# IrisRainbowNeko/HCP-Diffusion

Hardware: NVIDIA H100
Metric: LoRA-train images/sec SD1.5 512px (higher is better)
Workload: dtype bf16

## Files before the change

hcp_diffusion_b200/csrc/attention.cu:

```cuda
#include <stdlib.h>
#include "common.cuh"
#include "host_util.h"
#include "../../include/hcp_b200.h"

namespace hcp {

constexpr int kAttnThreads = 288;
constexpr int kAttnBwdThreads = 256;
constexpr int BOX_BYTES = 128 * 128;
constexpr float kLog2e = 1.4426950408889634f;
constexpr float kLn2 = 0.6931471805599453f;

__device__ __forceinline__ uint32_t kmajor_off(int ks, int box_bytes) { return (uint32_t)((ks >> 2) * (box_bytes >> 4) + (ks & 3) * 2); }
__device__ __forceinline__ float quad_max(float v) {
    v = fmaxf(v, __shfl_xor_sync(0xffffffffu, v, 1));
    return fmaxf(v, __shfl_xor_sync(0xffffffffu, v, 2));
}
__device__ __forceinline__ float quad_sum(float v) {
    v += __shfl_xor_sync(0xffffffffu, v, 1);
    return v + __shfl_xor_sync(0xffffffffu, v, 2);
}

struct alignas(64) AttnFwdParams {
    CUtensorMap tmQ, tmK, tmV;
    int B, H, Lq, Lkv, d;
    int nks;
    float scale_log2;
    const float* kv_bias;
    __nv_bfloat16* O;
    int64_t ldo;
    float* lse;
};

template <int NB, int KVT>
struct AttnFwdCfg {
    static constexpr int Q_BYTES = NB * BOX_BYTES;
    static constexpr int KV_BOX = KVT * 128;
    static constexpr int KV_BYTES = NB * KV_BOX;
    static constexpr int STAGES = 2;
    static constexpr int SMEM_BYTES = Q_BYTES + 2 * STAGES * KV_BYTES + 256 + 1024;
};

template <int NB, int KVT, bool kCausal>
__global__ void __launch_bounds__(kAttnThreads, 1) attn_fwd_kernel(const __grid_constant__ AttnFwdParams p) {
    using Cfg = AttnFwdCfg<NB, KVT>;
    constexpr int STAGES = Cfg::STAGES;
    constexpr int DN = 64 * NB;
    extern __shared__ uint8_t smem_raw[];
    uint8_t* smem = reinterpret_cast<uint8_t*>((reinterpret_cast<uintptr_t>(smem_raw) + 1023) & ~uintptr_t(1023));
    uint8_t* sQ = smem;
    uint8_t* sK = sQ + Cfg::Q_BYTES;
    uint8_t* sV = sK + STAGES * Cfg::KV_BYTES;
    uint64_t* bars = reinterpret_cast<uint64_t*>(sV + STAGES * Cfg::KV_BYTES);
    uint64_t* q_full = bars;
    uint64_t* kv_full = bars + 1;
    uint64_t* kv_empty = bars + 1 + STAGES;

    const int warp = warp_id_uniform(), lane = threadIdx.x & 31;
    const int qt = blockIdx.x, h = blockIdx.y, b = blockIdx.z;
    const int nkv = kCausal ? min((p.Lkv + KVT - 1) / KVT, (qt * 128 + 128 + KVT - 1) / KVT) : (p.Lkv + KVT - 1) / KVT;

    if (threadIdx.x == 0) {
        mbar_init(q_full, 1);
        for (int s = 0; s < STAGES; ++s) { mbar_init(&kv_full[s], 1); mbar_init(&kv_empty[s], 256); }
        fence_mbar_init();
    }
    __syncthreads();
    pdl_trigger();
    pdl_wait();

    if (warp == 8) {
        if (elect_one()) {
            mbar_arrive_expect_tx(q_full, Cfg::Q_BYTES);
            for (int bx = 0; bx < NB; ++bx) tma_load_4d(sQ + bx * BOX_BYTES, &p.tmQ, q_full, bx * 64, h, qt * 128, b);
            for (int j = 0; j < nkv; ++j) {
                const int st = j % STAGES;
                mbar_wait(&kv_empty[st], ((j / STAGES) & 1) ^ 1);
                mbar_arrive_expect_tx(&kv_full[st], 2 * Cfg::KV_BYTES);
                for (int bx = 0; bx < NB; ++bx) {
                    tma_load_4d(sK + st * Cfg::KV_BYTES + bx * Cfg::KV_BOX, &p.tmK, &kv_full[st], bx * 64, h, j * KVT, b);
                    tma_load_4d(sV + st * Cfg::KV_BYTES + bx * Cfg::KV_BOX, &p.tmV, &kv_full[st], bx * 64, h, j * KVT, b);
                }
            }
        }
        return;
    }

    const int wg = warp >> 2;
    const int g = lane >> 2, cq = 2 * (lane & 3);
    const int row0 = wg * 64 + (warp & 3) * 16 + g;
    const float* bias = p.kv_bias ? p.kv_bias + (int64_t)b * p.Lkv : nullptr;
    const float sl2 = p.scale_log2;
    float m[2] = {-INFINITY, -INFINITY}, l[2] = {0.f, 0.f};
    float o[DN / 2];
#pragma unroll
    for (int i = 0; i < DN / 2; ++i) o[i] = 0.f;
    const uint64_t qdesc = make_smem_desc(smem_u32(sQ) + wg * 64 * 128, 16, 1024);
    mbar_wait(q_full, 0);
    for (int j = 0; j < nkv; ++j) {
        const int st = j % STAGES;
        const int kv0 = j * KVT;
        const int ncols = min(KVT, p.Lkv - kv0);
        mbar_wait(&kv_full[st], (j / STAGES) & 1);
        float s[KVT / 2];
        const uint64_t kdesc = make_smem_desc(smem_u32(sK + st * Cfg::KV_BYTES), 16, 1024);
        wgmma_fence();
        wgmma_ss<KVT, 0, 0>(s, qdesc, kdesc, 0u);
        for (int ks = 1; ks < p.nks; ++ks)
            wgmma_ss<KVT, 0, 0>(s, desc_adv(qdesc, kmajor_off(ks, BOX_BYTES)), desc_adv(kdesc, kmajor_off(ks, Cfg::KV_BOX)), 1u);
        wgmma_commit();
        wgmma_wait<0>();
        wgmma_fence_acc(s);
        float mx[2] = {-INFINITY, -INFINITY};
        const bool diag = kCausal && kv0 + KVT > qt * 128;
#pragma unroll
        for (int c8 = 0; c8 < KVT / 8; ++c8) {
#pragma unroll
            for (int e = 0; e < 2; ++e) {
                const int col = c8 * 8 + cq + e;
                const float bv = (bias && col < ncols) ? bias[kv0 + col] * kLog2e : 0.f;
#pragma unroll
                for (int hh = 0; hh < 2; ++hh) {
                    float v = s[4 * c8 + 2 * hh + e] * sl2 + bv;
                    v = (col < ncols) ? v : -INFINITY;
                    if (diag && kv0 + col > qt * 128 + row0 + 8 * hh) v = -INFINITY;
                    s[4 * c8 + 2 * hh + e] = v;
                    mx[hh] = fmaxf(mx[hh], v);
                }
            }
        }
        float mu[2];
#pragma unroll
        for (int hh = 0; hh < 2; ++hh) {
            const float m_new = fmaxf(m[hh], quad_max(mx[hh]));
            mu[hh] = (m_new == -INFINITY) ? 0.f : m_new;
            const float alpha = fast_exp2(m[hh] - mu[hh]);
            l[hh] *= alpha;
#pragma unroll
            for (int c8 = 0; c8 < DN / 8; ++c8) { o[4 * c8 + 2 * hh] *= alpha; o[4 * c8 + 2 * hh + 1] *= alpha; }
            m[hh] = m_new;
        }
        uint32_t pa[KVT / 16][4];
#pragma unroll
        for (int kk = 0; kk < KVT / 16; ++kk) {
#pragma unroll
            for (int r = 0; r < 4; ++r) {
                const int hh = r & 1;
                const int i = 8 * kk + 4 * (r >> 1) + 2 * hh;
                const uint32_t u = pack_bf16x2(fast_exp2(s[i] - mu[hh]), fast_exp2(s[i + 1] - mu[hh]));
                const float2 f = unpack_bf16x2(u);
                l[hh] += f.x + f.y;
                pa[kk][r] = u;
            }
        }
        const uint64_t vdesc = make_smem_desc(smem_u32(sV + st * Cfg::KV_BYTES), Cfg::KV_BOX, 1024);
        wgmma_fence();
#pragma unroll
        for (int kk = 0; kk < KVT / 16; ++kk) wgmma_rs<DN, 1>(o, pa[kk], desc_adv(vdesc, kk * 128), 1u);
        wgmma_commit();
        wgmma_wait<0>();
        wgmma_fence_acc(o);
        mbar_arrive(&kv_empty[st]);
    }
#pragma unroll
    for (int hh = 0; hh < 2; ++hh) {
        const float lt = quad_sum(l[hh]);
        const int qrow = qt * 128 + row0 + 8 * hh;
        if (qrow >= p.Lq) continue;
        const float inv = 1.f / lt;
        __nv_bfloat16* orow = p.O + ((int64_t)b * p.Lq + qrow) * p.ldo + (int64_t)h * p.d;
#pragma unroll
        for (int c8 = 0; c8 < DN / 8; ++c8) {
            const int col = c8 * 8 + cq;
            if (col < p.d) *reinterpret_cast<uint32_t*>(orow + col) = pack_bf16x2(o[4 * c8 + 2 * hh] * inv, o[4 * c8 + 2 * hh + 1] * inv);
        }
        if (cq == 0 && p.lse) p.lse[((int64_t)b * p.H + h) * p.Lq + qrow] = ((m[hh] == -INFINITY ? 0.f : m[hh]) + log2f(lt)) * kLn2;
    }
}

struct alignas(64) AttnBwdParams {
    CUtensorMap tmQ, tmK, tmV, tmdO;
    int B, H, Lq, Lkv, d;
    int nks;
    int col0;
    float scale, scale_log2;
    const float* kv_bias;
    const float* stats;
    float* dq_acc;
    int dq_ld;
    int qsplit;
    float* dkv_acc;
    __nv_bfloat16 *dK, *dV;
    int64_t lddk, lddv;
};

template <int NB>
struct AttnBwdCfg {
    static constexpr int KV_BYTES = NB * BOX_BYTES;
    static constexpr int QBOX = 64 * 128;
    static constexpr int Q_BYTES = NB * QBOX;
    static constexpr int STAGES = 2;
    static constexpr int DS_BYTES = 64 * 128;
    static constexpr int STAT_BYTES = 2 * 64 * 4;
    static constexpr int SMEM_BYTES = 2 * KV_BYTES + 2 * STAGES * Q_BYTES + 2 * DS_BYTES + STAGES * STAT_BYTES + 256 + 1024;
};

template <int NB, bool kCausal>
__global__ void __launch_bounds__(kAttnBwdThreads, 1) attn_bwd_kernel(const __grid_constant__ AttnBwdParams p) {
    using Cfg = AttnBwdCfg<NB>;
    constexpr int STAGES = Cfg::STAGES;
    extern __shared__ uint8_t smem_raw[];
    uint8_t* smem = reinterpret_cast<uint8_t*>((reinterpret_cast<uintptr_t>(smem_raw) + 1023) & ~uintptr_t(1023));
    uint8_t* sK = smem;
    uint8_t* sV = sK + Cfg::KV_BYTES;
    uint8_t* sQ = sV + Cfg::KV_BYTES;
    uint8_t* sdO = sQ + STAGES * Cfg::Q_BYTES;
    uint8_t* sDS = sdO + STAGES * Cfg::Q_BYTES;
    uint8_t* sStat = sDS + 2 * Cfg::DS_BYTES;
    uint64_t* bars = reinterpret_cast<uint64_t*>(sStat + STAGES * Cfg::STAT_BYTES);
    uint64_t* kv_full = bars;
    uint64_t* q_full = bars + 1;

    const int warp = warp_id_uniform(), lane = threadIdx.x & 31;
    const int kt = blockIdx.x / p.qsplit, qs = blockIdx.x % p.qsplit;
    const int h = blockIdx.y, b = blockIdx.z;
    const int nq = (p.Lq + 63) / 64;
    const int per = 2 * (((nq + 1) / 2 + p.qsplit - 1) / p.qsplit);
    const int i0 = kCausal ? max(qs * per, 2 * kt) : qs * per, i1 = min(nq, qs * per + per);
    if (kCausal && i0 >= i1) return;
    const int64_t bh = (int64_t)b * p.H + h;

    if (threadIdx.x == 0) {
        mbar_init(kv_full, 1);
        for (int s = 0; s < STAGES; ++s) mbar_init(&q_full[s], 1);
        fence_mbar_init();
    }
    __syncthreads();
    pdl_trigger();
    pdl_wait();

    auto load_q = [&](int i) {
        const int st = (i - i0) % STAGES;
        mbar_arrive_expect_tx(&q_full[st], 2 * Cfg::Q_BYTES + Cfg::STAT_BYTES);
        for (int bx = 0; bx < NB; ++bx) {
            tma_load_4d(sQ + st * Cfg::Q_BYTES + bx * Cfg::QBOX, &p.tmQ, &q_full[st], bx * 64, h, i * 64, b);
            tma_load_4d(sdO + st * Cfg::Q_BYTES + bx * Cfg::QBOX, &p.tmdO, &q_full[st], bx * 64, h, i * 64, b);
        }
        bulk_load(sStat + st * Cfg::STAT_BYTES, p.stats + (bh * nq + i) * 128, Cfg::STAT_BYTES, &q_full[st]);
    };
    if (threadIdx.x == 0) {
        mbar_arrive_expect_tx(kv_full, 2 * Cfg::KV_BYTES);
        for (int bx = 0; bx < NB; ++bx) {
            tma_load_4d(sK + bx * BOX_BYTES, &p.tmK, kv_full, bx * 64, h, kt * 128, b);
            tma_load_4d(sV + bx * BOX_BYTES, &p.tmV, kv_full, bx * 64, h, kt * 128, b);
        }
        for (int i = i0; i < min(i1, i0 + STAGES); ++i) load_q(i);
    }

    const int wg = warp >> 2;
    const int g = lane >> 2, cq = 2 * (lane & 3);
    const int r0 = (warp & 3) * 16 + g;
    const int kvw = kt * 128 + wg * 64;
    const float sl2 = p.scale_log2, scale = p.scale;
    const int cbox = p.col0 / 64;
    float kvb[2];
    bool kv_ok[2];
#pragma unroll
    for (int hh = 0; hh < 2; ++hh) {
        const int kv = kvw + r0 + 8 * hh;
        kv_ok[hh] = kv < p.Lkv;
        kvb[hh] = (p.kv_bias && kv_ok[hh]) ? p.kv_bias[(int64_t)b * p.Lkv + kv] * kLog2e : 0.f;
    }
    float dv[32], dk[32];
#pragma unroll
    for (int i = 0; i < 32; ++i) { dv[i] = 0.f; dk[i] = 0.f; }
    const uint64_t kdesc = make_smem_desc(smem_u32(sK) + wg * 64 * 128, 16, 1024);
    const uint64_t vdesc = make_smem_desc(smem_u32(sV) + wg * 64 * 128, 16, 1024);
    const int dq_col = p.col0 + 32 * wg;
    const bool dq_cols = dq_col < p.d;
    const uint64_t kdesc_mn = make_smem_desc(smem_u32(sK) + cbox * BOX_BYTES + wg * 64, BOX_BYTES, 1024);
    const uint32_t ds_base = smem_u32(sDS) + wg * Cfg::DS_BYTES;
    const uint64_t dsdesc = make_smem_desc(smem_u32(sDS), 2 * Cfg::DS_BYTES, 1024);
    mbar_wait(kv_full, 0);
    for (int i = i0; i < i1; ++i) {
        const int st = (i - i0) % STAGES;
        mbar_wait(&q_full[st], ((i - i0) / STAGES) & 1);
        const uint32_t qb = smem_u32(sQ + st * Cfg::Q_BYTES), dob = smem_u32(sdO + st * Cfg::Q_BYTES);
        const uint32_t statb = smem_u32(sStat + st * Cfg::STAT_BYTES);
        const uint64_t qdesc = make_smem_desc(qb, 16, 1024), dodesc = make_smem_desc(dob, 16, 1024);
        float s[32], dp[32];
        wgmma_fence();
        wgmma_ss<64, 0, 0>(s, kdesc, qdesc, 0u);
        for (int ks = 1; ks < p.nks; ++ks)
            wgmma_ss<64, 0, 0>(s, desc_adv(kdesc, kmajor_off(ks, BOX_BYTES)), desc_adv(qdesc, kmajor_off(ks, Cfg::QBOX)), 1u);
        wgmma_ss<64, 0, 0>(dp, vdesc, dodesc, 0u);
        for (int ks = 1; ks < p.nks; ++ks)
            wgmma_ss<64, 0, 0>(dp, desc_adv(vdesc, kmajor_off(ks, BOX_BYTES)), desc_adv(dodesc, kmajor_off(ks, Cfg::QBOX)), 1u);
        wgmma_commit();
        wgmma_wait<0>();
        wgmma_fence_acc(s);
        wgmma_fence_acc(dp);
        uint32_t pa[4][4], da[4][4];
        const bool diag = kCausal && i < 2 * kt + 2;
#pragma unroll
        for (int kk = 0; kk < 4; ++kk) {
            float lq[4], dq_[4];
#pragma unroll
            for (int c2 = 0; c2 < 2; ++c2) {
                const uint32_t a = statb + (16 * kk + 8 * c2 + cq) * 4;
                const float2 l2 = lds_f32x2(a), d2 = lds_f32x2(a + 64 * 4);
                lq[2 * c2] = l2.x; lq[2 * c2 + 1] = l2.y;
                dq_[2 * c2] = d2.x; dq_[2 * c2 + 1] = d2.y;
            }
#pragma unroll
            for (int r = 0; r < 4; ++r) {
                const int hh = r & 1;
                const int c = 2 * (r >> 1);
                const int idx = 8 * kk + 4 * (r >> 1) + 2 * hh;
                float pv[2], dsv[2];
#pragma unroll
                for (int e = 0; e < 2; ++e) {
                    float pe = kv_ok[hh] ? fast_exp2(s[idx + e] * sl2 + kvb[hh] - lq[c + e]) : 0.f;
                    if (diag && kvw + r0 + 8 * hh > i * 64 + 16 * kk + 8 * (r >> 1) + cq + e) pe = 0.f;
                    pv[e] = pe;
                    dsv[e] = scale * pe * (dp[idx + e] - dq_[c + e]);
                }
                pa[kk][r] = pack_bf16x2(pv[0], pv[1]);
                da[kk][r] = pack_bf16x2(dsv[0], dsv[1]);
                const int row = r0 + 8 * hh, col = 16 * kk + 8 * (r >> 1) + cq;
                asm volatile("st.shared.b32 [%0], %1;" ::"r"(ds_base + sw128_offset(row, col >> 3) + (col & 7) * 2), "r"(da[kk][r]) : "memory");
            }
        }
        fence_proxy_async_smem();
        asm volatile("bar.sync 1, 256;" ::: "memory");
        const uint64_t dodesc_mn = make_smem_desc(dob + cbox * Cfg::QBOX, Cfg::QBOX, 1024);
        const uint64_t qdesc_mn = make_smem_desc(qb + cbox * Cfg::QBOX, Cfg::QBOX, 1024);
        float dqa[16];
        wgmma_fence();
#pragma unroll
        for (int kk = 0; kk < 4; ++kk) wgmma_rs<64, 1>(dv, pa[kk], desc_adv(dodesc_mn, kk * 128), 1u);
#pragma unroll
        for (int kk = 0; kk < 4; ++kk) wgmma_rs<64, 1>(dk, da[kk], desc_adv(qdesc_mn, kk * 128), 1u);
        if (dq_cols) {
            wgmma_ss<32, 1, 1>(dqa, dsdesc, kdesc_mn, 0u);
#pragma unroll
            for (int kk = 1; kk < 8; ++kk) wgmma_ss<32, 1, 1>(dqa, desc_adv(dsdesc, kk * 128), desc_adv(kdesc_mn, kk * 128), 1u);
        }
        wgmma_commit();
        wgmma_wait<0>();
        wgmma_fence_acc(dv);
        wgmma_fence_acc(dk);
        wgmma_fence_acc(dqa);
        asm volatile("bar.sync 1, 256;" ::: "memory");
        if (threadIdx.x == 0 && i + STAGES < i1) load_q(i + STAGES);
        if (!dq_cols) continue;
#pragma unroll
        for (int hh = 0; hh < 2; ++hh) {
            const int q = i * 64 + r0 + 8 * hh;
            if (q >= p.Lq) continue;
#pragma unroll
            for (int c8 = 0; c8 < 4; ++c8) {
                const int col = dq_col + 8 * c8 + cq;
                if (col < p.d) red_add_v2(p.dq_acc + ((bh * (p.dq_ld / 4) + col / 4) * p.Lq + q) * 4 + (col & 3), dqa[4 * c8 + 2 * hh], dqa[4 * c8 + 2 * hh + 1]);
            }
        }
    }
#pragma unroll
    for (int hh = 0; hh < 2; ++hh) {
        if (!kv_ok[hh]) continue;
        const int kv = kvw + r0 + 8 * hh;
#pragma unroll
        for (int c8 = 0; c8 < 8; ++c8) {
            const int col = p.col0 + 8 * c8 + cq;
            if (col >= p.d) continue;
            const float v0 = dv[4 * c8 + 2 * hh], v1 = dv[4 * c8 + 2 * hh + 1];
            const float k0 = dk[4 * c8 + 2 * hh], k1 = dk[4 * c8 + 2 * hh + 1];
            if (p.dkv_acc) {
                float* base = p.dkv_acc + ((bh * p.Lkv + kv) * 2) * p.dq_ld + col;
                red_add_v2(base, v0, v1);
                red_add_v2(base + p.dq_ld, k0, k1);
            } else {
                *reinterpret_cast<uint32_t*>(p.dV + ((int64_t)b * p.Lkv + kv) * p.lddv + (int64_t)h * p.d + col) = pack_bf16x2(v0, v1);
                *reinterpret_cast<uint32_t*>(p.dK + ((int64_t)b * p.Lkv + kv) * p.lddk + (int64_t)h * p.d + col) = pack_bf16x2(k0, k1);
            }
        }
    }
}

__global__ void __launch_bounds__(256) attn_bwd_prep_kernel(const __nv_bfloat16* __restrict__ O, int64_t ldo,
                                                            const __nv_bfloat16* __restrict__ dO, int64_t lddo,
                                                            const float* __restrict__ lse, int B, int H, int Lq, int d,
                                                            float* __restrict__ stats, float* __restrict__ dq_acc,
                                                            int64_t dq_n, float* __restrict__ dkv_acc, int64_t dkv_n) {
    pdl_trigger();
    pdl_wait();
    const int64_t gtid = blockIdx.x * (int64_t)blockDim.x + threadIdx.x;
    const int64_t nthreads = (int64_t)gridDim.x * blockDim.x;
    if (dq_acc) {
        float4* z = reinterpret_cast<float4*>(dq_acc);
        for (int64_t i = gtid; i < dq_n / 4; i += nthreads) z[i] = make_float4(0.f, 0.f, 0.f, 0.f);
    }
    if (dkv_acc) {
        float4* z = reinterpret_cast<float4*>(dkv_acc);
        for (int64_t i = gtid; i < dkv_n / 4; i += nthreads) z[i] = make_float4(0.f, 0.f, 0.f, 0.f);
    }
    const int nq = (Lq + 63) / 64;
    const int64_t total = (int64_t)B * nq * 64 * H;
    if (gtid >= total) return;
    const int h = (int)(gtid % H);
    const int64_t bq = gtid / H;
    const int q = (int)(bq % (nq * 64));
    const int b = (int)(bq / (nq * 64));
    float* st = stats + (((int64_t)b * H + h) * nq + q / 64) * 128 + (q & 63);
    if (q >= Lq) {
        st[0] = INFINITY;
        st[64] = 0.f;
        return;
    }
    const int64_t row = (int64_t)b * Lq + q;
    const uint4* o = reinterpret_cast<const uint4*>(O + row * ldo + (int64_t)h * d);
    const uint4* g = reinterpret_cast<const uint4*>(dO + row * lddo + (int64_t)h * d);
    float acc = 0.f;
    for (int e = 0; e < d / 8; ++e) {
        const uint4 a = o[e], c = g[e];
        float2 x, y;
        x = unpack_bf16x2(a.x); y = unpack_bf16x2(c.x); acc += x.x * y.x + x.y * y.y;
        x = unpack_bf16x2(a.y); y = unpack_bf16x2(c.y); acc += x.x * y.x + x.y * y.y;
        x = unpack_bf16x2(a.z); y = unpack_bf16x2(c.z); acc += x.x * y.x + x.y * y.y;
        x = unpack_bf16x2(a.w); y = unpack_bf16x2(c.w); acc += x.x * y.x + x.y * y.y;
    }
    st[0] = lse[((int64_t)b * H + h) * Lq + q] * kLog2e;
    st[64] = acc;
}

__global__ void attn_bwd_post_kernel(const float* __restrict__ dq_acc, int dq_ld, int B, int H, int Lq, int d,
                                     __nv_bfloat16* __restrict__ dQ, int64_t lddq) {
    pdl_trigger();
    pdl_wait();
    const int64_t i = blockIdx.x * (int64_t)blockDim.x + threadIdx.x;
    const int d4 = d / 4;
    const int64_t total = (int64_t)B * Lq * H * d4;
    if (i >= total) return;
    const int e = (int)(i % d4) * 4;
    const int64_t r = i / d4;
    const int h = (int)(r % H);
    const int64_t bq = r / H;
    const int q = (int)(bq % Lq);
    const int b = (int)(bq / Lq);
    const float4 v = *reinterpret_cast<const float4*>(dq_acc + ((((int64_t)b * H + h) * (dq_ld / 4) + e / 4) * Lq + q) * 4);
    uint2 o;
    o.x = pack_bf16x2(v.x, v.y);
    o.y = pack_bf16x2(v.z, v.w);
    *reinterpret_cast<uint2*>(dQ + bq * lddq + (int64_t)h * d + e) = o;
}

__global__ void attn_bwd_post_kv_kernel(const float* __restrict__ acc, int dq_ld, int B, int H, int Lkv, int d,
                                        __nv_bfloat16* __restrict__ dK, int64_t lddk, __nv_bfloat16* __restrict__ dV, int64_t lddv) {
    pdl_trigger();
    pdl_wait();
    const int64_t i = blockIdx.x * (int64_t)blockDim.x + threadIdx.x;
    const int d4 = d / 4;
    const int64_t total = (int64_t)B * Lkv * H * 2 * d4;
    if (i >= total) return;
    const int e = (int)(i % d4) * 4;
    int64_t r = i / d4;
    const int which = (int)(r % 2); r /= 2;
    const int h = (int)(r % H);
    const int64_t bk = r / H;
    const int kv = (int)(bk % Lkv);
    const int b = (int)(bk / Lkv);
    const float4 v = *reinterpret_cast<const float4*>(acc + ((((int64_t)b * H + h) * Lkv + kv) * 2 + which) * dq_ld + e);
    uint2 o;
    o.x = pack_bf16x2(v.x, v.y);
    o.y = pack_bf16x2(v.z, v.w);
    __nv_bfloat16* dst = which ? dK : dV;
    const int64_t ld = which ? lddk : lddv;
    *reinterpret_cast<uint2*>(dst + bk * ld + (int64_t)h * d + e) = o;
}

static int make_head_map(CUtensorMap* m, const void* base, int64_t ld, int64_t B, int64_t H, int64_t L, int64_t d, uint32_t rows) {
    uint64_t dims[4] = {(uint64_t)d, (uint64_t)H, (uint64_t)L, (uint64_t)B};
    uint64_t strides[3] = {(uint64_t)d * 2, (uint64_t)ld * 2, (uint64_t)L * ld * 2};
    uint32_t box[4] = {64, 1, rows, 1};
    return make_tmap_nd(m, base, 4, dims, strides, box);
}

static int check_common(int64_t B, int64_t H, int64_t Lq, int64_t Lkv, int64_t d) {
    if (B <= 0 || H <= 0 || Lq <= 0 || Lkv <= 0) return set_error(HCP_ERR_INVALID, "attention: empty problem");
    if (d % 8 != 0 || d < 8 || d > 192) return set_error(HCP_ERR_INVALID, "attention: head dim must be a multiple of 8 in [8,192]");
    return HCP_OK;
}

template <int NB, int KVT, bool kCausal>
static int launch_attn_fwd(const AttnFwdParams& p, dim3 grid, cudaStream_t stream) {
    using Cfg = AttnFwdCfg<NB, KVT>;
    static bool configured = false;
    if (!configured) {
        cudaError_t e = cudaFuncSetAttribute(attn_fwd_kernel<NB, KVT, kCausal>, cudaFuncAttributeMaxDynamicSharedMemorySize, Cfg::SMEM_BYTES);
        if (e != cudaSuccess) return set_cuda_error(e, "cudaFuncSetAttribute(attn_fwd)");
        configured = true;
    }
    launch_k(attn_fwd_kernel<NB, KVT, kCausal>, grid, dim3(kAttnThreads), Cfg::SMEM_BYTES, stream, p);
    cudaError_t e = cudaGetLastError();
    if (e != cudaSuccess) return set_cuda_error(e, "attn_fwd launch");
    return HCP_OK;
}

template <int NB, bool kCausal>
static int launch_attn_bwd(const AttnBwdParams& p, dim3 grid, cudaStream_t stream) {
    using Cfg = AttnBwdCfg<NB>;
    static bool configured = false;
    if (!configured) {
        cudaError_t e = cudaFuncSetAttribute(attn_bwd_kernel<NB, kCausal>, cudaFuncAttributeMaxDynamicSharedMemorySize, Cfg::SMEM_BYTES);
        if (e != cudaSuccess) return set_cuda_error(e, "cudaFuncSetAttribute(attn_bwd)");
        configured = true;
    }
    launch_k(attn_bwd_kernel<NB, kCausal>, grid, dim3(kAttnBwdThreads), Cfg::SMEM_BYTES, stream, p);
    cudaError_t e = cudaGetLastError();
    if (e != cudaSuccess) return set_cuda_error(e, "attn_bwd launch");
    return HCP_OK;
}

}

using namespace hcp;

template <bool kCausal>
static int attn_fwd(const hcp_attn_args* a, hcp_stream_t stream_) {
    if (!a || !a->q || !a->k || !a->v || !a->o) return set_error(HCP_ERR_INVALID, "attn_fwd: null pointer");
    int rc = check_common(a->B, a->H, a->Lq, a->Lkv, a->d);
    if (rc) return rc;
    if (kCausal && a->Lq != a->Lkv) return set_error(HCP_ERR_INVALID, "attn_fwd_causal: Lq must equal Lkv");
    const int nb = (int)((a->d + 63) / 64);
    const uint32_t kvt = nb == 3 ? 64 : 128;
    AttnFwdParams p;
    memset(&p, 0, sizeof(p));
    if ((rc = make_head_map(&p.tmQ, a->q, a->ldq, a->B, a->H, a->Lq, a->d, 128))) return rc;
    if ((rc = make_head_map(&p.tmK, a->k, a->ldk, a->B, a->H, a->Lkv, a->d, kvt))) return rc;
    if ((rc = make_head_map(&p.tmV, a->v, a->ldv, a->B, a->H, a->Lkv, a->d, kvt))) return rc;
    p.B = (int)a->B; p.H = (int)a->H; p.Lq = (int)a->Lq; p.Lkv = (int)a->Lkv; p.d = (int)a->d;
    p.nks = (int)((a->d + 15) / 16);
    p.scale_log2 = a->scale * kLog2e;
    p.kv_bias = a->kv_bias;
    p.O = (__nv_bfloat16*)a->o; p.ldo = a->ldo;
    p.lse = a->lse;
    const dim3 grid((unsigned)((a->Lq + 127) / 128), (unsigned)a->H, (unsigned)a->B);
    cudaStream_t stream = (cudaStream_t)stream_;
    if (nb == 1) return launch_attn_fwd<1, 128, kCausal>(p, grid, stream);
    if (nb == 2) return launch_attn_fwd<2, 128, kCausal>(p, grid, stream);
    return launch_attn_fwd<3, 64, kCausal>(p, grid, stream);
}

extern "C" int hcp_attn_fwd_bf16(const hcp_attn_args* a, hcp_stream_t stream) { return attn_fwd<false>(a, stream); }
extern "C" int hcp_attn_fwd_causal_bf16(const hcp_attn_args* a, hcp_stream_t stream) { return attn_fwd<true>(a, stream); }

static int plan_qsplit(int64_t B, int64_t H, int64_t Lq, int64_t Lkv) {
    const int64_t base = ((Lkv + 127) / 128) * H * B;
    const int64_t nq = (Lq + 127) / 128;
    const int64_t sms = num_sms();
    if (base >= sms * 4 / 5 || nq < 2) return 1;
    int64_t qs = (2 * sms + base - 1) / base;
    if (qs > nq) qs = nq;
    const int64_t per = (nq + qs - 1) / qs;
    return (int)((nq + per - 1) / per);
}

extern "C" size_t hcp_attn_bwd_workspace_bytes(int64_t B, int64_t H, int64_t Lq, int64_t Lkv, int64_t d) {
    const int64_t dq_ld = (d + 3) / 4 * 4;
    size_t n = (size_t)(B * H * ((Lq + 63) / 64) * 128) + (size_t)(B * H * Lq * dq_ld);
    if (plan_qsplit(B, H, Lq, Lkv) > 1) n += (size_t)(B * H * Lkv * 2 * dq_ld);
    return n * sizeof(float);
}

template <bool kCausal>
static int attn_bwd(const hcp_attn_bwd_args* a, hcp_stream_t stream_) {
    if (!a || !a->q || !a->k || !a->v || !a->o || !a->dout || !a->lse || !a->dq || !a->dk || !a->dv || !a->workspace)
        return set_error(HCP_ERR_INVALID, "attn_bwd: null pointer");
    int rc = check_common(a->B, a->H, a->Lq, a->Lkv, a->d);
    if (rc) return rc;
    if (kCausal && a->Lq != a->Lkv) return set_error(HCP_ERR_INVALID, "attn_bwd_causal: Lq must equal Lkv");
    if (a->workspace_bytes < hcp_attn_bwd_workspace_bytes(a->B, a->H, a->Lq, a->Lkv, a->d))
        return set_error(HCP_ERR_INVALID, "attn_bwd: workspace too small");
    if ((a->ldo % 8) != 0 || (a->lddo % 8) != 0 || (a->lddq % 8) != 0) return set_error(HCP_ERR_INVALID, "attn_bwd: leading dimensions must be multiples of 8");
    cudaStream_t stream = (cudaStream_t)stream_;
    const int dq_ld = (int)((a->d + 3) / 4 * 4);
    float* stats = a->workspace;
    float* dq_acc = a->workspace + a->B * a->H * ((a->Lq + 63) / 64) * 128;
    const int qsplit = plan_qsplit(a->B, a->H, a->Lq, a->Lkv);
    const int64_t dkv_n = qsplit > 1 ? a->B * a->H * a->Lkv * 2 * dq_ld : 0;
    float* dkv_acc = qsplit > 1 ? dq_acc + a->B * a->H * a->Lq * dq_ld : nullptr;
    {
        const int64_t total = a->B * ((a->Lq + 63) / 64 * 64) * a->H;
        const int threads = 256;
        const int64_t blocks = (total + threads - 1) / threads;
        launch_k(attn_bwd_prep_kernel, dim3((unsigned)blocks), dim3(threads), 0, stream, (const __nv_bfloat16*)a->o, a->ldo,
                 (const __nv_bfloat16*)a->dout, a->lddo, (const float*)a->lse, (int)a->B, (int)a->H, (int)a->Lq, (int)a->d, stats,
                 dq_acc, (int64_t)(a->B * a->H * a->Lq * dq_ld), dkv_acc, dkv_n);
    }
    AttnBwdParams p;
    memset(&p, 0, sizeof(p));
    if ((rc = make_head_map(&p.tmQ, a->q, a->ldq, a->B, a->H, a->Lq, a->d, 64))) return rc;
    if ((rc = make_head_map(&p.tmK, a->k, a->ldk, a->B, a->H, a->Lkv, a->d, 128))) return rc;
    if ((rc = make_head_map(&p.tmV, a->v, a->ldv, a->B, a->H, a->Lkv, a->d, 128))) return rc;
    if ((rc = make_head_map(&p.tmdO, a->dout, a->lddo, a->B, a->H, a->Lq, a->d, 64))) return rc;
    p.B = (int)a->B; p.H = (int)a->H; p.Lq = (int)a->Lq; p.Lkv = (int)a->Lkv; p.d = (int)a->d;
    p.nks = (int)((a->d + 15) / 16);
    p.scale = a->scale;
    p.scale_log2 = a->scale * kLog2e;
    p.kv_bias = a->kv_bias;
    p.stats = stats;
    p.dq_acc = dq_acc;
    p.dq_ld = dq_ld;
    p.qsplit = qsplit;
    p.dkv_acc = dkv_acc;
    p.dK = (__nv_bfloat16*)a->dk; p.lddk = a->lddk;
    p.dV = (__nv_bfloat16*)a->dv; p.lddv = a->lddv;
    const int nb = (int)((a->d + 63) / 64);
    const dim3 grid((unsigned)(((a->Lkv + 127) / 128) * qsplit), (unsigned)a->H, (unsigned)a->B);
    for (int col0 = 0; col0 < a->d; col0 += 64) {
        p.col0 = col0;
        rc = nb == 1 ? launch_attn_bwd<1, kCausal>(p, grid, stream) : nb == 2 ? launch_attn_bwd<2, kCausal>(p, grid, stream)
                     : launch_attn_bwd<3, kCausal>(p, grid, stream);
        if (rc) return rc;
    }
    {
        const int64_t n = a->B * a->Lq * a->H * (a->d / 4);
        launch_k(attn_bwd_post_kernel, dim3((unsigned)((n + 255) / 256)), dim3(256), 0, stream, dq_acc, dq_ld, (int)a->B, (int)a->H, (int)a->Lq,
                 (int)a->d, (__nv_bfloat16*)a->dq, a->lddq);
    }
    if (qsplit > 1) {
        const int64_t n = a->B * a->Lkv * a->H * 2 * (a->d / 4);
        launch_k(attn_bwd_post_kv_kernel, dim3((unsigned)((n + 255) / 256)), dim3(256), 0, stream, dkv_acc, dq_ld, (int)a->B, (int)a->H, (int)a->Lkv, (int)a->d,
                                                                                (__nv_bfloat16*)a->dk, a->lddk, (__nv_bfloat16*)a->dv, a->lddv);
    }
    cudaError_t e = cudaGetLastError();
    if (e != cudaSuccess) return set_cuda_error(e, "attn_bwd post launch");
    return HCP_OK;
}

extern "C" int hcp_attn_bwd_bf16(const hcp_attn_bwd_args* a, hcp_stream_t stream) { return attn_bwd<false>(a, stream); }
extern "C" int hcp_attn_bwd_causal_bf16(const hcp_attn_bwd_args* a, hcp_stream_t stream) { return attn_bwd<true>(a, stream); }
```

hcp_diffusion_b200/csrc/wgmma.cuh:

```cuda
#pragma once
#include <stdint.h>

namespace hcp {
template <int TA, int TB>
__device__ __forceinline__ void wgmma_ss_n32(float (&d)[16], uint64_t a, uint64_t b, uint32_t accumulate) {
    asm volatile(
        "{\n\t.reg .pred p;\n\t"
        "setp.ne.b32 p, %18, 0;\n\t"
        "wgmma.mma_async.sync.aligned.m64n32k16.f32.bf16.bf16 "
        "{%0, %1, %2, %3, %4, %5, %6, %7, %8, %9, %10, %11, %12, %13, %14, %15}, "
        "%16, %17, p, 1, 1, %19, %20;\n\t}"
        : "+f"(d[0]), "+f"(d[1]), "+f"(d[2]), "+f"(d[3]), "+f"(d[4]), "+f"(d[5]), "+f"(d[6]), "+f"(d[7]), "+f"(d[8]), "+f"(d[9]), "+f"(d[10]), "+f"(d[11]), "+f"(d[12]), "+f"(d[13]), "+f"(d[14]), "+f"(d[15])
        : "l"(a), "l"(b), "r"(accumulate), "n"(TA), "n"(TB));
}
template <int TA, int TB>
__device__ __forceinline__ void wgmma_ss_n64(float (&d)[32], uint64_t a, uint64_t b, uint32_t accumulate) {
    asm volatile(
        "{\n\t.reg .pred p;\n\t"
        "setp.ne.b32 p, %34, 0;\n\t"
        "wgmma.mma_async.sync.aligned.m64n64k16.f32.bf16.bf16 "
        "{%0, %1, %2, %3, %4, %5, %6, %7, %8, %9, %10, %11, %12, %13, %14, %15, %16, %17, %18, %19, %20, %21, %22, %23, %24, %25, %26, %27, %28, %29, %30, %31}, "
        "%32, %33, p, 1, 1, %35, %36;\n\t}"
        : "+f"(d[0]), "+f"(d[1]), "+f"(d[2]), "+f"(d[3]), "+f"(d[4]), "+f"(d[5]), "+f"(d[6]), "+f"(d[7]), "+f"(d[8]), "+f"(d[9]), "+f"(d[10]), "+f"(d[11]), "+f"(d[12]), "+f"(d[13]), "+f"(d[14]), "+f"(d[15]), "+f"(d[16]), "+f"(d[17]), "+f"(d[18]), "+f"(d[19]), "+f"(d[20]), "+f"(d[21]), "+f"(d[22]), "+f"(d[23]), "+f"(d[24]), "+f"(d[25]), "+f"(d[26]), "+f"(d[27]), "+f"(d[28]), "+f"(d[29]), "+f"(d[30]), "+f"(d[31])
        : "l"(a), "l"(b), "r"(accumulate), "n"(TA), "n"(TB));
}
template <int TA, int TB>
__device__ __forceinline__ void wgmma_ss_n128(float (&d)[64], uint64_t a, uint64_t b, uint32_t accumulate) {
    asm volatile(
        "{\n\t.reg .pred p;\n\t"
        "setp.ne.b32 p, %66, 0;\n\t"
        "wgmma.mma_async.sync.aligned.m64n128k16.f32.bf16.bf16 "
        "{%0, %1, %2, %3, %4, %5, %6, %7, %8, %9, %10, %11, %12, %13, %14, %15, %16, %17, %18, %19, %20, %21, %22, %23, %24, %25, %26, %27, %28, %29, %30, %31, %32, %33, %34, %35, %36, %37, %38, %39, %40, %41, %42, %43, %44, %45, %46, %47, %48, %49, %50, %51, %52, %53, %54, %55, %56, %57, %58, %59, %60, %61, %62, %63}, "
        "%64, %65, p, 1, 1, %67, %68;\n\t}"
        : "+f"(d[0]), "+f"(d[1]), "+f"(d[2]), "+f"(d[3]), "+f"(d[4]), "+f"(d[5]), "+f"(d[6]), "+f"(d[7]), "+f"(d[8]), "+f"(d[9]), "+f"(d[10]), "+f"(d[11]), "+f"(d[12]), "+f"(d[13]), "+f"(d[14]), "+f"(d[15]), "+f"(d[16]), "+f"(d[17]), "+f"(d[18]), "+f"(d[19]), "+f"(d[20]), "+f"(d[21]), "+f"(d[22]), "+f"(d[23]), "+f"(d[24]), "+f"(d[25]), "+f"(d[26]), "+f"(d[27]), "+f"(d[28]), "+f"(d[29]), "+f"(d[30]), "+f"(d[31]), "+f"(d[32]), "+f"(d[33]), "+f"(d[34]), "+f"(d[35]), "+f"(d[36]), "+f"(d[37]), "+f"(d[38]), "+f"(d[39]), "+f"(d[40]), "+f"(d[41]), "+f"(d[42]), "+f"(d[43]), "+f"(d[44]), "+f"(d[45]), "+f"(d[46]), "+f"(d[47]), "+f"(d[48]), "+f"(d[49]), "+f"(d[50]), "+f"(d[51]), "+f"(d[52]), "+f"(d[53]), "+f"(d[54]), "+f"(d[55]), "+f"(d[56]), "+f"(d[57]), "+f"(d[58]), "+f"(d[59]), "+f"(d[60]), "+f"(d[61]), "+f"(d[62]), "+f"(d[63])
        : "l"(a), "l"(b), "r"(accumulate), "n"(TA), "n"(TB));
}
template <int TA, int TB>
__device__ __forceinline__ void wgmma_ss_n160(float (&d)[80], uint64_t a, uint64_t b, uint32_t accumulate) {
    asm volatile(
        "{\n\t.reg .pred p;\n\t"
        "setp.ne.b32 p, %82, 0;\n\t"
        "wgmma.mma_async.sync.aligned.m64n160k16.f32.bf16.bf16 "
        "{%0, %1, %2, %3, %4, %5, %6, %7, %8, %9, %10, %11, %12, %13, %14, %15, %16, %17, %18, %19, %20, %21, %22, %23, %24, %25, %26, %27, %28, %29, %30, %31, %32, %33, %34, %35, %36, %37, %38, %39, %40, %41, %42, %43, %44, %45, %46, %47, %48, %49, %50, %51, %52, %53, %54, %55, %56, %57, %58, %59, %60, %61, %62, %63, %64, %65, %66, %67, %68, %69, %70, %71, %72, %73, %74, %75, %76, %77, %78, %79}, "
        "%80, %81, p, 1, 1, %83, %84;\n\t}"
        : "+f"(d[0]), "+f"(d[1]), "+f"(d[2]), "+f"(d[3]), "+f"(d[4]), "+f"(d[5]), "+f"(d[6]), "+f"(d[7]), "+f"(d[8]), "+f"(d[9]), "+f"(d[10]), "+f"(d[11]), "+f"(d[12]), "+f"(d[13]), "+f"(d[14]), "+f"(d[15]), "+f"(d[16]), "+f"(d[17]), "+f"(d[18]), "+f"(d[19]), "+f"(d[20]), "+f"(d[21]), "+f"(d[22]), "+f"(d[23]), "+f"(d[24]), "+f"(d[25]), "+f"(d[26]), "+f"(d[27]), "+f"(d[28]), "+f"(d[29]), "+f"(d[30]), "+f"(d[31]), "+f"(d[32]), "+f"(d[33]), "+f"(d[34]), "+f"(d[35]), "+f"(d[36]), "+f"(d[37]), "+f"(d[38]), "+f"(d[39]), "+f"(d[40]), "+f"(d[41]), "+f"(d[42]), "+f"(d[43]), "+f"(d[44]), "+f"(d[45]), "+f"(d[46]), "+f"(d[47]), "+f"(d[48]), "+f"(d[49]), "+f"(d[50]), "+f"(d[51]), "+f"(d[52]), "+f"(d[53]), "+f"(d[54]), "+f"(d[55]), "+f"(d[56]), "+f"(d[57]), "+f"(d[58]), "+f"(d[59]), "+f"(d[60]), "+f"(d[61]), "+f"(d[62]), "+f"(d[63]), "+f"(d[64]), "+f"(d[65]), "+f"(d[66]), "+f"(d[67]), "+f"(d[68]), "+f"(d[69]), "+f"(d[70]), "+f"(d[71]), "+f"(d[72]), "+f"(d[73]), "+f"(d[74]), "+f"(d[75]), "+f"(d[76]), "+f"(d[77]), "+f"(d[78]), "+f"(d[79])
        : "l"(a), "l"(b), "r"(accumulate), "n"(TA), "n"(TB));
}
template <int TA, int TB>
__device__ __forceinline__ void wgmma_ss_n176(float (&d)[88], uint64_t a, uint64_t b, uint32_t accumulate) {
    asm volatile(
        "{\n\t.reg .pred p;\n\t"
        "setp.ne.b32 p, %90, 0;\n\t"
        "wgmma.mma_async.sync.aligned.m64n176k16.f32.bf16.bf16 "
        "{%0, %1, %2, %3, %4, %5, %6, %7, %8, %9, %10, %11, %12, %13, %14, %15, %16, %17, %18, %19, %20, %21, %22, %23, %24, %25, %26, %27, %28, %29, %30, %31, %32, %33, %34, %35, %36, %37, %38, %39, %40, %41, %42, %43, %44, %45, %46, %47, %48, %49, %50, %51, %52, %53, %54, %55, %56, %57, %58, %59, %60, %61, %62, %63, %64, %65, %66, %67, %68, %69, %70, %71, %72, %73, %74, %75, %76, %77, %78, %79, %80, %81, %82, %83, %84, %85, %86, %87}, "
        "%88, %89, p, 1, 1, %91, %92;\n\t}"
        : "+f"(d[0]), "+f"(d[1]), "+f"(d[2]), "+f"(d[3]), "+f"(d[4]), "+f"(d[5]), "+f"(d[6]), "+f"(d[7]), "+f"(d[8]), "+f"(d[9]), "+f"(d[10]), "+f"(d[11]), "+f"(d[12]), "+f"(d[13]), "+f"(d[14]), "+f"(d[15]), "+f"(d[16]), "+f"(d[17]), "+f"(d[18]), "+f"(d[19]), "+f"(d[20]), "+f"(d[21]), "+f"(d[22]), "+f"(d[23]), "+f"(d[24]), "+f"(d[25]), "+f"(d[26]), "+f"(d[27]), "+f"(d[28]), "+f"(d[29]), "+f"(d[30]), "+f"(d[31]), "+f"(d[32]), "+f"(d[33]), "+f"(d[34]), "+f"(d[35]), "+f"(d[36]), "+f"(d[37]), "+f"(d[38]), "+f"(d[39]), "+f"(d[40]), "+f"(d[41]), "+f"(d[42]), "+f"(d[43]), "+f"(d[44]), "+f"(d[45]), "+f"(d[46]), "+f"(d[47]), "+f"(d[48]), "+f"(d[49]), "+f"(d[50]), "+f"(d[51]), "+f"(d[52]), "+f"(d[53]), "+f"(d[54]), "+f"(d[55]), "+f"(d[56]), "+f"(d[57]), "+f"(d[58]), "+f"(d[59]), "+f"(d[60]), "+f"(d[61]), "+f"(d[62]), "+f"(d[63]), "+f"(d[64]), "+f"(d[65]), "+f"(d[66]), "+f"(d[67]), "+f"(d[68]), "+f"(d[69]), "+f"(d[70]), "+f"(d[71]), "+f"(d[72]), "+f"(d[73]), "+f"(d[74]), "+f"(d[75]), "+f"(d[76]), "+f"(d[77]), "+f"(d[78]), "+f"(d[79]), "+f"(d[80]), "+f"(d[81]), "+f"(d[82]), "+f"(d[83]), "+f"(d[84]), "+f"(d[85]), "+f"(d[86]), "+f"(d[87])
        : "l"(a), "l"(b), "r"(accumulate), "n"(TA), "n"(TB));
}
template <int TB>
__device__ __forceinline__ void wgmma_rs_n64(float (&d)[32], const uint32_t (&a)[4], uint64_t b, uint32_t accumulate) {
    asm volatile(
        "{\n\t.reg .pred p;\n\t"
        "setp.ne.b32 p, %37, 0;\n\t"
        "wgmma.mma_async.sync.aligned.m64n64k16.f32.bf16.bf16 "
        "{%0, %1, %2, %3, %4, %5, %6, %7, %8, %9, %10, %11, %12, %13, %14, %15, %16, %17, %18, %19, %20, %21, %22, %23, %24, %25, %26, %27, %28, %29, %30, %31}, "
        "{%32, %33, %34, %35}, %36, p, 1, 1, %38;\n\t}"
        : "+f"(d[0]), "+f"(d[1]), "+f"(d[2]), "+f"(d[3]), "+f"(d[4]), "+f"(d[5]), "+f"(d[6]), "+f"(d[7]), "+f"(d[8]), "+f"(d[9]), "+f"(d[10]), "+f"(d[11]), "+f"(d[12]), "+f"(d[13]), "+f"(d[14]), "+f"(d[15]), "+f"(d[16]), "+f"(d[17]), "+f"(d[18]), "+f"(d[19]), "+f"(d[20]), "+f"(d[21]), "+f"(d[22]), "+f"(d[23]), "+f"(d[24]), "+f"(d[25]), "+f"(d[26]), "+f"(d[27]), "+f"(d[28]), "+f"(d[29]), "+f"(d[30]), "+f"(d[31])
        : "r"(a[0]), "r"(a[1]), "r"(a[2]), "r"(a[3]), "l"(b), "r"(accumulate), "n"(TB));
}
template <int TB>
__device__ __forceinline__ void wgmma_rs_n128(float (&d)[64], const uint32_t (&a)[4], uint64_t b, uint32_t accumulate) {
    asm volatile(
        "{\n\t.reg .pred p;\n\t"
        "setp.ne.b32 p, %69, 0;\n\t"
        "wgmma.mma_async.sync.aligned.m64n128k16.f32.bf16.bf16 "
        "{%0, %1, %2, %3, %4, %5, %6, %7, %8, %9, %10, %11, %12, %13, %14, %15, %16, %17, %18, %19, %20, %21, %22, %23, %24, %25, %26, %27, %28, %29, %30, %31, %32, %33, %34, %35, %36, %37, %38, %39, %40, %41, %42, %43, %44, %45, %46, %47, %48, %49, %50, %51, %52, %53, %54, %55, %56, %57, %58, %59, %60, %61, %62, %63}, "
        "{%64, %65, %66, %67}, %68, p, 1, 1, %70;\n\t}"
        : "+f"(d[0]), "+f"(d[1]), "+f"(d[2]), "+f"(d[3]), "+f"(d[4]), "+f"(d[5]), "+f"(d[6]), "+f"(d[7]), "+f"(d[8]), "+f"(d[9]), "+f"(d[10]), "+f"(d[11]), "+f"(d[12]), "+f"(d[13]), "+f"(d[14]), "+f"(d[15]), "+f"(d[16]), "+f"(d[17]), "+f"(d[18]), "+f"(d[19]), "+f"(d[20]), "+f"(d[21]), "+f"(d[22]), "+f"(d[23]), "+f"(d[24]), "+f"(d[25]), "+f"(d[26]), "+f"(d[27]), "+f"(d[28]), "+f"(d[29]), "+f"(d[30]), "+f"(d[31]), "+f"(d[32]), "+f"(d[33]), "+f"(d[34]), "+f"(d[35]), "+f"(d[36]), "+f"(d[37]), "+f"(d[38]), "+f"(d[39]), "+f"(d[40]), "+f"(d[41]), "+f"(d[42]), "+f"(d[43]), "+f"(d[44]), "+f"(d[45]), "+f"(d[46]), "+f"(d[47]), "+f"(d[48]), "+f"(d[49]), "+f"(d[50]), "+f"(d[51]), "+f"(d[52]), "+f"(d[53]), "+f"(d[54]), "+f"(d[55]), "+f"(d[56]), "+f"(d[57]), "+f"(d[58]), "+f"(d[59]), "+f"(d[60]), "+f"(d[61]), "+f"(d[62]), "+f"(d[63])
        : "r"(a[0]), "r"(a[1]), "r"(a[2]), "r"(a[3]), "l"(b), "r"(accumulate), "n"(TB));
}
template <int TB>
__device__ __forceinline__ void wgmma_rs_n192(float (&d)[96], const uint32_t (&a)[4], uint64_t b, uint32_t accumulate) {
    asm volatile(
        "{\n\t.reg .pred p;\n\t"
        "setp.ne.b32 p, %101, 0;\n\t"
        "wgmma.mma_async.sync.aligned.m64n192k16.f32.bf16.bf16 "
        "{%0, %1, %2, %3, %4, %5, %6, %7, %8, %9, %10, %11, %12, %13, %14, %15, %16, %17, %18, %19, %20, %21, %22, %23, %24, %25, %26, %27, %28, %29, %30, %31, %32, %33, %34, %35, %36, %37, %38, %39, %40, %41, %42, %43, %44, %45, %46, %47, %48, %49, %50, %51, %52, %53, %54, %55, %56, %57, %58, %59, %60, %61, %62, %63, %64, %65, %66, %67, %68, %69, %70, %71, %72, %73, %74, %75, %76, %77, %78, %79, %80, %81, %82, %83, %84, %85, %86, %87, %88, %89, %90, %91, %92, %93, %94, %95}, "
        "{%96, %97, %98, %99}, %100, p, 1, 1, %102;\n\t}"
        : "+f"(d[0]), "+f"(d[1]), "+f"(d[2]), "+f"(d[3]), "+f"(d[4]), "+f"(d[5]), "+f"(d[6]), "+f"(d[7]), "+f"(d[8]), "+f"(d[9]), "+f"(d[10]), "+f"(d[11]), "+f"(d[12]), "+f"(d[13]), "+f"(d[14]), "+f"(d[15]), "+f"(d[16]), "+f"(d[17]), "+f"(d[18]), "+f"(d[19]), "+f"(d[20]), "+f"(d[21]), "+f"(d[22]), "+f"(d[23]), "+f"(d[24]), "+f"(d[25]), "+f"(d[26]), "+f"(d[27]), "+f"(d[28]), "+f"(d[29]), "+f"(d[30]), "+f"(d[31]), "+f"(d[32]), "+f"(d[33]), "+f"(d[34]), "+f"(d[35]), "+f"(d[36]), "+f"(d[37]), "+f"(d[38]), "+f"(d[39]), "+f"(d[40]), "+f"(d[41]), "+f"(d[42]), "+f"(d[43]), "+f"(d[44]), "+f"(d[45]), "+f"(d[46]), "+f"(d[47]), "+f"(d[48]), "+f"(d[49]), "+f"(d[50]), "+f"(d[51]), "+f"(d[52]), "+f"(d[53]), "+f"(d[54]), "+f"(d[55]), "+f"(d[56]), "+f"(d[57]), "+f"(d[58]), "+f"(d[59]), "+f"(d[60]), "+f"(d[61]), "+f"(d[62]), "+f"(d[63]), "+f"(d[64]), "+f"(d[65]), "+f"(d[66]), "+f"(d[67]), "+f"(d[68]), "+f"(d[69]), "+f"(d[70]), "+f"(d[71]), "+f"(d[72]), "+f"(d[73]), "+f"(d[74]), "+f"(d[75]), "+f"(d[76]), "+f"(d[77]), "+f"(d[78]), "+f"(d[79]), "+f"(d[80]), "+f"(d[81]), "+f"(d[82]), "+f"(d[83]), "+f"(d[84]), "+f"(d[85]), "+f"(d[86]), "+f"(d[87]), "+f"(d[88]), "+f"(d[89]), "+f"(d[90]), "+f"(d[91]), "+f"(d[92]), "+f"(d[93]), "+f"(d[94]), "+f"(d[95])
        : "r"(a[0]), "r"(a[1]), "r"(a[2]), "r"(a[3]), "l"(b), "r"(accumulate), "n"(TB));
}
template <int N, int TA, int TB>
__device__ __forceinline__ void wgmma_ss(float (&d)[N / 2], uint64_t a, uint64_t b, uint32_t accumulate) {
    if constexpr (N == 32) wgmma_ss_n32<TA, TB>(d, a, b, accumulate);
    else if constexpr (N == 64) wgmma_ss_n64<TA, TB>(d, a, b, accumulate);
    else if constexpr (N == 128) wgmma_ss_n128<TA, TB>(d, a, b, accumulate);
    else if constexpr (N == 160) wgmma_ss_n160<TA, TB>(d, a, b, accumulate);
    else if constexpr (N == 176) wgmma_ss_n176<TA, TB>(d, a, b, accumulate);
    else static_assert(N == 0, "wgmma_ss: unsupported N");
}
template <int N, int TB>
__device__ __forceinline__ void wgmma_rs(float (&d)[N / 2], const uint32_t (&a)[4], uint64_t b, uint32_t accumulate) {
    if constexpr (N == 64) wgmma_rs_n64<TB>(d, a, b, accumulate);
    else if constexpr (N == 128) wgmma_rs_n128<TB>(d, a, b, accumulate);
    else if constexpr (N == 192) wgmma_rs_n192<TB>(d, a, b, accumulate);
    else static_assert(N == 0, "wgmma_rs: unsupported N");
}

__device__ __forceinline__ void wgmma_fence() { asm volatile("wgmma.fence.sync.aligned;" ::: "memory"); }
__device__ __forceinline__ void wgmma_commit() { asm volatile("wgmma.commit_group.sync.aligned;" ::: "memory"); }
template <int N>
__device__ __forceinline__ void wgmma_wait() { asm volatile("wgmma.wait_group.sync.aligned %0;" ::"n"(N) : "memory"); }
template <int R>
__device__ __forceinline__ void wgmma_fence_acc(float (&d)[R]) {
#pragma unroll
    for (int i = 0; i < R; ++i) asm volatile("" : "+f"(d[i])::"memory");
}

}
```

Measured before the change: 105.1.

## Software-pipeline attention fwd/bwd and trim wgmma N to head dim

The forward kernel drops the dedicated producer warp, issues TMA loads from thread 0, and uses three KV stages. It overlaps the QK^T wgmma of tile j with the PV wgmma of tile j-1, and folds the softmax scale into the exp2 on full tiles. The backward kernel splits S and dP into separate commit groups and overlaps the dV wgmma with the dS computation. A template width SW/DN sizes the O/dV/dK accumulators to the real head dimension (40, 80, 160 for SD1.5) rather than multiples of 64, with new wgmma N variants generated by macros and optional clock64 tracing. This trades extra shared memory and register pressure, plus more complex ordering, for less tensor-core idle time and fewer wasted MMA columns.

```diff
diff --git a/hcp_diffusion_b200/csrc/attention.cu b/hcp_diffusion_b200/csrc/attention.cu
--- a/hcp_diffusion_b200/csrc/attention.cu
+++ b/hcp_diffusion_b200/csrc/attention.cu
@@ -5,13 +5,35 @@
 
 namespace hcp {
 
-constexpr int kAttnThreads = 288;
+constexpr int kAttnThreads = 256;
 constexpr int kAttnBwdThreads = 256;
 constexpr int BOX_BYTES = 128 * 128;
 constexpr float kLog2e = 1.4426950408889634f;
 constexpr float kLn2 = 0.6931471805599453f;
 
 __device__ __forceinline__ uint32_t kmajor_off(int ks, int box_bytes) { return (uint32_t)((ks >> 2) * (box_bytes >> 4) + (ks & 3) * 2); }
+constexpr int kTracePhases = 9;
+#ifdef HCP_ATTN_TRACE
+__device__ unsigned long long g_attn_trace[2][kTracePhases + 1];
+#define ATTN_TRACE_INIT()                 \
+    long long tr_[kTracePhases] = {};     \
+    long long tr_t = clock64()
+#define ATTN_TRACE(ph)                    \
+    do {                                  \
+        const long long t_ = clock64();   \
+        tr_[ph] += t_ - tr_t;             \
+        tr_t = t_;                        \
+    } while (0)
+#define ATTN_TRACE_FLUSH(kernel, iters)                                                                                          \
+    if ((threadIdx.x & 127) == 0) {                                                                                              \
+        for (int k_ = 0; k_ < kTracePhases; ++k_) atomicAdd(&g_attn_trace[kernel][k_], (unsigned long long)tr_[k_]);             \
+        atomicAdd(&g_attn_trace[kernel][kTracePhases], (unsigned long long)(iters));                                             \
+    }
+#else
+#define ATTN_TRACE_INIT() ((void)0)
+#define ATTN_TRACE(ph) ((void)0)
+#define ATTN_TRACE_FLUSH(kernel, iters) ((void)0)
+#endif
 __device__ __forceinline__ float quad_max(float v) {
     v = fmaxf(v, __shfl_xor_sync(0xffffffffu, v, 1));
     return fmaxf(v, __shfl_xor_sync(0xffffffffu, v, 2));
@@ -37,15 +59,16 @@
     static constexpr int Q_BYTES = NB * BOX_BYTES;
     static constexpr int KV_BOX = KVT * 128;
     static constexpr int KV_BYTES = NB * KV_BOX;
-    static constexpr int STAGES = 2;
+    static constexpr int STAGES = 3;
     static constexpr int SMEM_BYTES = Q_BYTES + 2 * STAGES * KV_BYTES + 256 + 1024;
+    static_assert(SMEM_BYTES <= 227 * 1024, "attn_fwd: shared memory");
 };
 
-template <int NB, int KVT, bool kCausal>
+template <int NB, int KVT, int DN, bool kCausal>
 __global__ void __launch_bounds__(kAttnThreads, 1) attn_fwd_kernel(const __grid_constant__ AttnFwdParams p) {
     using Cfg = AttnFwdCfg<NB, KVT>;
     constexpr int STAGES = Cfg::STAGES;
-    constexpr int DN = 64 * NB;
+    static_assert(DN <= 64 * NB && DN > 64 * (NB - 1), "attn_fwd: O width");
     extern __shared__ uint8_t smem_raw[];
     uint8_t* smem = reinterpret_cast<uint8_t*>((reinterpret_cast<uintptr_t>(smem_raw) + 1023) & ~uintptr_t(1023));
     uint8_t* sQ = smem;
@@ -69,21 +92,19 @@
     pdl_trigger();
     pdl_wait();
 
-    if (warp == 8) {
-        if (elect_one()) {
-            mbar_arrive_expect_tx(q_full, Cfg::Q_BYTES);
-            for (int bx = 0; bx < NB; ++bx) tma_load_4d(sQ + bx * BOX_BYTES, &p.tmQ, q_full, bx * 64, h, qt * 128, b);
-            for (int j = 0; j < nkv; ++j) {
-                const int st = j % STAGES;
-                mbar_wait(&kv_empty[st], ((j / STAGES) & 1) ^ 1);
-                mbar_arrive_expect_tx(&kv_full[st], 2 * Cfg::KV_BYTES);
-                for (int bx = 0; bx < NB; ++bx) {
-                    tma_load_4d(sK + st * Cfg::KV_BYTES + bx * Cfg::KV_BOX, &p.tmK, &kv_full[st], bx * 64, h, j * KVT, b);
-                    tma_load_4d(sV + st * Cfg::KV_BYTES + bx * Cfg::KV_BOX, &p.tmV, &kv_full[st], bx * 64, h, j * KVT, b);
-                }
-            }
-        }
-        return;
+    auto load_kv = [&](int j) {
+        const int st = j % STAGES;
+        mbar_wait(&kv_empty[st], ((j / STAGES) & 1) ^ 1);
+        mbar_arrive_expect_tx(&kv_full[st], 2 * Cfg::KV_BYTES);
+        for (int bx = 0; bx < NB; ++bx) {
+            tma_load_4d(sK + st * Cfg::KV_BYTES + bx * Cfg::KV_BOX, &p.tmK, &kv_full[st], bx * 64, h, j * KVT, b);
+            tma_load_4d(sV + st * Cfg::KV_BYTES + bx * Cfg::KV_BOX, &p.tmV, &kv_full[st], bx * 64, h, j * KVT, b);
+        }
+    };
+    if (threadIdx.x == 0) {
+        mbar_arrive_expect_tx(q_full, Cfg::Q_BYTES);
+        for (int bx = 0; bx < NB; ++bx) tma_load_4d(sQ + bx * BOX_BYTES, &p.tmQ, q_full, bx * 64, h, qt * 128, b);
+        for (int j = 0; j < min(nkv, STAGES); ++j) load_kv(j);
     }
 
     const int wg = warp >> 2;
@@ -96,36 +117,52 @@
 #pragma unroll
     for (int i = 0; i < DN / 2; ++i) o[i] = 0.f;
     const uint64_t qdesc = make_smem_desc(smem_u32(sQ) + wg * 64 * 128, 16, 1024);
-    mbar_wait(q_full, 0);
-    for (int j = 0; j < nkv; ++j) {
-        const int st = j % STAGES;
-        const int kv0 = j * KVT;
-        const int ncols = min(KVT, p.Lkv - kv0);
-        mbar_wait(&kv_full[st], (j / STAGES) & 1);
-        float s[KVT / 2];
-        const uint64_t kdesc = make_smem_desc(smem_u32(sK + st * Cfg::KV_BYTES), 16, 1024);
-        wgmma_fence();
+    float s[KVT / 2];
+    auto issue_s = [&](int j) {
+        const uint64_t kdesc = make_smem_desc(smem_u32(sK + (j % STAGES) * Cfg::KV_BYTES), 16, 1024);
         wgmma_ss<KVT, 0, 0>(s, qdesc, kdesc, 0u);
         for (int ks = 1; ks < p.nks; ++ks)
             wgmma_ss<KVT, 0, 0>(s, desc_adv(qdesc, kmajor_off(ks, BOX_BYTES)), desc_adv(kdesc, kmajor_off(ks, Cfg::KV_BOX)), 1u);
         wgmma_commit();
-        wgmma_wait<0>();
+    };
+    uint32_t pa[KVT / 16][4];
+    auto issue_pv = [&](int j) {
+        const uint64_t vdesc = make_smem_desc(smem_u32(sV + (j % STAGES) * Cfg::KV_BYTES), Cfg::KV_BOX, 1024);
+#pragma unroll
+        for (int kk = 0; kk < KVT / 16; ++kk) wgmma_rs<DN, 1>(o, pa[kk], desc_adv(vdesc, kk * 128), 1u);
+        wgmma_commit();
+    };
+    float alpha[2];
+    auto softmax_tile = [&](int j) {
+        const int kv0 = j * KVT;
+        const int ncols = min(KVT, p.Lkv - kv0);
         wgmma_fence_acc(s);
         float mx[2] = {-INFINITY, -INFINITY};
         const bool diag = kCausal && kv0 + KVT > qt * 128;
-#pragma unroll
-        for (int c8 = 0; c8 < KVT / 8; ++c8) {
-#pragma unroll
-            for (int e = 0; e < 2; ++e) {
-                const int col = c8 * 8 + cq + e;
-                const float bv = (bias && col < ncols) ? bias[kv0 + col] * kLog2e : 0.f;
-#pragma unroll
-                for (int hh = 0; hh < 2; ++hh) {
-                    float v = s[4 * c8 + 2 * hh + e] * sl2 + bv;
-                    v = (col < ncols) ? v : -INFINITY;
-                    if (diag && kv0 + col > qt * 128 + row0 + 8 * hh) v = -INFINITY;
-                    s[4 * c8 + 2 * hh + e] = v;
-                    mx[hh] = fmaxf(mx[hh], v);
+        const bool folded = bias == nullptr && ncols == KVT && !diag && sl2 > 0.f;
+        if (folded) {
+#pragma unroll
+            for (int c8 = 0; c8 < KVT / 8; ++c8) {
+                mx[0] = fmaxf(mx[0], fmaxf(s[4 * c8], s[4 * c8 + 1]));
+                mx[1] = fmaxf(mx[1], fmaxf(s[4 * c8 + 2], s[4 * c8 + 3]));
+            }
+            mx[0] *= sl2;
+            mx[1] *= sl2;
+        } else {
+#pragma unroll
+            for (int c8 = 0; c8 < KVT / 8; ++c8) {
+#pragma unroll
+                for (int e = 0; e < 2; ++e) {
+                    const int col = c8 * 8 + cq + e;
+                    const float bv = (bias && col < ncols) ? bias[kv0 + col] * kLog2e : 0.f;
+#pragma unroll
+                    for (int hh = 0; hh < 2; ++hh) {
+                        float v = s[4 * c8 + 2 * hh + e] * sl2 + bv;
+                        v = (col < ncols) ? v : -INFINITY;
+                        if (diag && kv0 + col > qt * 128 + row0 + 8 * hh) v = -INFINITY;
+                        s[4 * c8 + 2 * hh + e] = v;
+                        mx[hh] = fmaxf(mx[hh], v);
+                    }
                 }
             }
         }
@@ -134,34 +171,66 @@
         for (int hh = 0; hh < 2; ++hh) {
             const float m_new = fmaxf(m[hh], quad_max(mx[hh]));
             mu[hh] = (m_new == -INFINITY) ? 0.f : m_new;
-            const float alpha = fast_exp2(m[hh] - mu[hh]);
-            l[hh] *= alpha;
-#pragma unroll
-            for (int c8 = 0; c8 < DN / 8; ++c8) { o[4 * c8 + 2 * hh] *= alpha; o[4 * c8 + 2 * hh + 1] *= alpha; }
+            alpha[hh] = fast_exp2(m[hh] - mu[hh]);
             m[hh] = m_new;
         }
-        uint32_t pa[KVT / 16][4];
+        const float fs = folded ? sl2 : 1.f;
+#pragma unroll
+        for (int i = 0; i < KVT / 2; ++i) s[i] = fast_exp2(fmaf(s[i], fs, -mu[(i >> 1) & 1]));
+    };
+    auto rescale_pack = [&]() {
+#pragma unroll
+        for (int hh = 0; hh < 2; ++hh) {
+            l[hh] *= alpha[hh];
+#pragma unroll
+            for (int c8 = 0; c8 < DN / 8; ++c8) { o[4 * c8 + 2 * hh] *= alpha[hh]; o[4 * c8 + 2 * hh + 1] *= alpha[hh]; }
+        }
 #pragma unroll
         for (int kk = 0; kk < KVT / 16; ++kk) {
 #pragma unroll
             for (int r = 0; r < 4; ++r) {
                 const int hh = r & 1;
                 const int i = 8 * kk + 4 * (r >> 1) + 2 * hh;
-                const uint32_t u = pack_bf16x2(fast_exp2(s[i] - mu[hh]), fast_exp2(s[i + 1] - mu[hh]));
+                const uint32_t u = pack_bf16x2(s[i], s[i + 1]);
                 const float2 f = unpack_bf16x2(u);
                 l[hh] += f.x + f.y;
                 pa[kk][r] = u;
             }
         }
-        const uint64_t vdesc = make_smem_desc(smem_u32(sV + st * Cfg::KV_BYTES), Cfg::KV_BOX, 1024);
+    };
+    ATTN_TRACE_INIT();
+    mbar_wait(q_full, 0);
+    mbar_wait(&kv_full[0], 0);
+    wgmma_fence();
+    issue_s(0);
+    wgmma_wait<0>();
+    softmax_tile(0);
+    rescale_pack();
+    ATTN_TRACE(5);
+    for (int j = 1; j < nkv; ++j) {
+        if (threadIdx.x == 0 && j >= STAGES - 1 && j + 1 < nkv) load_kv(j + 1);
+        mbar_wait(&kv_full[j % STAGES], (j / STAGES) & 1);
         wgmma_fence();
-#pragma unroll
-        for (int kk = 0; kk < KVT / 16; ++kk) wgmma_rs<DN, 1>(o, pa[kk], desc_adv(vdesc, kk * 128), 1u);
-        wgmma_commit();
+        issue_s(j);
+        issue_pv(j - 1);
+        ATTN_TRACE(0);
+        wgmma_wait<1>();
+        ATTN_TRACE(1);
+        softmax_tile(j);
+        ATTN_TRACE(2);
         wgmma_wait<0>();
         wgmma_fence_acc(o);
-        mbar_arrive(&kv_empty[st]);
-    }
+        ATTN_TRACE(3);
+        mbar_arrive(&kv_empty[(j - 1) % STAGES]);
+        rescale_pack();
+        ATTN_TRACE(4);
+    }
+    wgmma_fence();
+    issue_pv(nkv - 1);
+    wgmma_wait<0>();
+    wgmma_fence_acc(o);
+    ATTN_TRACE(5);
+    ATTN_TRACE_FLUSH(0, nkv - 1);
 #pragma unroll
     for (int hh = 0; hh < 2; ++hh) {
         const float lt = quad_sum(l[hh]);
@@ -205,7 +274,7 @@
     static constexpr int SMEM_BYTES = 2 * KV_BYTES + 2 * STAGES * Q_BYTES + 2 * DS_BYTES + STAGES * STAT_BYTES + 256 + 1024;
 };
 
-template <int NB, bool kCausal>
+template <int NB, int SW, bool kCausal>
 __global__ void __launch_bounds__(kAttnBwdThreads, 1) attn_bwd_kernel(const __grid_constant__ AttnBwdParams p) {
     using Cfg = AttnBwdCfg<NB>;
     constexpr int STAGES = Cfg::STAGES;
@@ -271,106 +340,164 @@
         kv_ok[hh] = kv < p.Lkv;
         kvb[hh] = (p.kv_bias && kv_ok[hh]) ? p.kv_bias[(int64_t)b * p.Lkv + kv] * kLog2e : 0.f;
     }
-    float dv[32], dk[32];
-#pragma unroll
-    for (int i = 0; i < 32; ++i) { dv[i] = 0.f; dk[i] = 0.f; }
+    float dv[SW / 2], dk[SW / 2];
+#pragma unroll
+    for (int i = 0; i < SW / 2; ++i) { dv[i] = 0.f; dk[i] = 0.f; }
     const uint64_t kdesc = make_smem_desc(smem_u32(sK) + wg * 64 * 128, 16, 1024);
     const uint64_t vdesc = make_smem_desc(smem_u32(sV) + wg * 64 * 128, 16, 1024);
-    const int dq_col = p.col0 + 32 * wg;
+    constexpr int H0 = SW == 40 ? 32 : SW / 2;
+    constexpr int H1A = (SW > 64 ? 64 : SW) - H0, H1B = SW - H0 - H1A;
+    const int dq_col = p.col0 + (wg ? H0 : 0);
     const bool dq_cols = dq_col < p.d;
-    const uint64_t kdesc_mn = make_smem_desc(smem_u32(sK) + cbox * BOX_BYTES + wg * 64, BOX_BYTES, 1024);
+    const uint64_t kdesc_mn = make_smem_desc(smem_u32(sK) + cbox * BOX_BYTES + (wg ? 2 * H0 : 0), BOX_BYTES, 1024);
+    const uint64_t kdesc_mn_b = make_smem_desc(smem_u32(sK) + (cbox + 1) * BOX_BYTES, BOX_BYTES, 1024);
     const uint32_t ds_base = smem_u32(sDS) + wg * Cfg::DS_BYTES;
     const uint64_t dsdesc = make_smem_desc(smem_u32(sDS), 2 * Cfg::DS_BYTES, 1024);
-    mbar_wait(kv_full, 0);
-    for (int i = i0; i < i1; ++i) {
+    float s[32], dp[32];
+    auto issue_sdp = [&](int i) {
         const int st = (i - i0) % STAGES;
         mbar_wait(&q_full[st], ((i - i0) / STAGES) & 1);
-        const uint32_t qb = smem_u32(sQ + st * Cfg::Q_BYTES), dob = smem_u32(sdO + st * Cfg::Q_BYTES);
-        const uint32_t statb = smem_u32(sStat + st * Cfg::STAT_BYTES);
-        const uint64_t qdesc = make_smem_desc(qb, 16, 1024), dodesc = make_smem_desc(dob, 16, 1024);
-        float s[32], dp[32];
+        const uint64_t qdesc = make_smem_desc(smem_u32(sQ + st * Cfg::Q_BYTES), 16, 1024);
+        const uint64_t dodesc = make_smem_desc(smem_u32(sdO + st * Cfg::Q_BYTES), 16, 1024);
         wgmma_fence();
         wgmma_ss<64, 0, 0>(s, kdesc, qdesc, 0u);
         for (int ks = 1; ks < p.nks; ++ks)
             wgmma_ss<64, 0, 0>(s, desc_adv(kdesc, kmajor_off(ks, BOX_BYTES)), desc_adv(qdesc, kmajor_off(ks, Cfg::QBOX)), 1u);
+        wgmma_commit();
         wgmma_ss<64, 0, 0>(dp, vdesc, dodesc, 0u);
         for (int ks = 1; ks < p.nks; ++ks)
             wgmma_ss<64, 0, 0>(dp, desc_adv(vdesc, kmajor_off(ks, BOX_BYTES)), desc_adv(dodesc, kmajor_off(ks, Cfg::QBOX)), 1u);
         wgmma_commit();
-        wgmma_wait<0>();
+    };
+    ATTN_TRACE_INIT();
+    mbar_wait(kv_full, 0);
+    for (int i = i0; i < i1; ++i) {
+        const int st = (i - i0) % STAGES;
+        ATTN_TRACE(8);
+        issue_sdp(i);
+        ATTN_TRACE(0);
+        const uint32_t qb = smem_u32(sQ + st * Cfg::Q_BYTES), dob = smem_u32(sdO + st * Cfg::Q_BYTES);
+        const uint32_t statb = smem_u32(sStat + st * Cfg::STAT_BYTES);
+        const uint64_t dodesc_mn = make_smem_desc(dob + cbox * Cfg::QBOX, Cfg::QBOX, 1024);
+        const uint64_t qdesc_mn = make_smem_desc(qb + cbox * Cfg::QBOX, Cfg::QBOX, 1024);
+        wgmma_wait<1>();
         wgmma_fence_acc(s);
-        wgmma_fence_acc(dp);
+        ATTN_TRACE(1);
         uint32_t pa[4][4], da[4][4];
         const bool diag = kCausal && i < 2 * kt + 2;
 #pragma unroll
         for (int kk = 0; kk < 4; ++kk) {
-            float lq[4], dq_[4];
+            float lq[4];
 #pragma unroll
             for (int c2 = 0; c2 < 2; ++c2) {
-                const uint32_t a = statb + (16 * kk + 8 * c2 + cq) * 4;
-                const float2 l2 = lds_f32x2(a), d2 = lds_f32x2(a + 64 * 4);
+                const float2 l2 = lds_f32x2(statb + (16 * kk + 8 * c2 + cq) * 4);
                 lq[2 * c2] = l2.x; lq[2 * c2 + 1] = l2.y;
-                dq_[2 * c2] = d2.x; dq_[2 * c2 + 1] = d2.y;
             }
 #pragma unroll
             for (int r = 0; r < 4; ++r) {
                 const int hh = r & 1;
                 const int c = 2 * (r >> 1);
                 const int idx = 8 * kk + 4 * (r >> 1) + 2 * hh;
-                float pv[2], dsv[2];
 #pragma unroll
                 for (int e = 0; e < 2; ++e) {
                     float pe = kv_ok[hh] ? fast_exp2(s[idx + e] * sl2 + kvb[hh] - lq[c + e]) : 0.f;
                     if (diag && kvw + r0 + 8 * hh > i * 64 + 16 * kk + 8 * (r >> 1) + cq + e) pe = 0.f;
-                    pv[e] = pe;
-                    dsv[e] = scale * pe * (dp[idx + e] - dq_[c + e]);
+                    s[idx + e] = pe;
                 }
-                pa[kk][r] = pack_bf16x2(pv[0], pv[1]);
-                da[kk][r] = pack_bf16x2(dsv[0], dsv[1]);
+                pa[kk][r] = pack_bf16x2(s[idx], s[idx + 1]);
+            }
+        }
+        ATTN_TRACE(2);
+        wgmma_fence();
+#pragma unroll
+        for (int kk = 0; kk < 4; ++kk) wgmma_rs<SW, 1>(dv, pa[kk], desc_adv(dodesc_mn, kk * 128), 1u);
+        wgmma_commit();
+        wgmma_wait<1>();
+        wgmma_fence_acc(dp);
+        ATTN_TRACE(3);
+#pragma unroll
+        for (int kk = 0; kk < 4; ++kk) {
+            float dq_[4];
+#pragma unroll
+            for (int c2 = 0; c2 < 2; ++c2) {
+                const float2 d2 = lds_f32x2(statb + (64 + 16 * kk + 8 * c2 + cq) * 4);
+                dq_[2 * c2] = d2.x; dq_[2 * c2 + 1] = d2.y;
+            }
+#pragma unroll
+            for (int r = 0; r < 4; ++r) {
+                const int hh = r & 1;
+                const int c = 2 * (r >> 1);
+                const int idx = 8 * kk + 4 * (r >> 1) + 2 * hh;
+                da[kk][r] = pack_bf16x2(scale * s[idx] * (dp[idx] - dq_[c]), scale * s[idx + 1] * (dp[idx + 1] - dq_[c + 1]));
                 const int row = r0 + 8 * hh, col = 16 * kk + 8 * (r >> 1) + cq;
                 asm volatile("st.shared.b32 [%0], %1;" ::"r"(ds_base + sw128_offset(row, col >> 3) + (col & 7) * 2), "r"(da[kk][r]) : "memory");
             }
         }
         fence_proxy_async_smem();
+        ATTN_TRACE(4);
         asm volatile("bar.sync 1, 256;" ::: "memory");
-        const uint64_t dodesc_mn = make_smem_desc(dob + cbox * Cfg::QBOX, Cfg::QBOX, 1024);
-        const uint64_t qdesc_mn = make_smem_desc(qb + cbox * Cfg::QBOX, Cfg::QBOX, 1024);
-        float dqa[16];
+        ATTN_TRACE(5);
+        float dqa[H0 / 2], dqa_a[H1A / 2], dqa_b[H1B > 0 ? H1B / 2 : 1];
         wgmma_fence();
 #pragma unroll
-        for (int kk = 0; kk < 4; ++kk) wgmma_rs<64, 1>(dv, pa[kk], desc_adv(dodesc_mn, kk * 128), 1u);
-#pragma unroll
-        for (int kk = 0; kk < 4; ++kk) wgmma_rs<64, 1>(dk, da[kk], desc_adv(qdesc_mn, kk * 128), 1u);
-        if (dq_cols) {
-            wgmma_ss<32, 1, 1>(dqa, dsdesc, kdesc_mn, 0u);
-#pragma unroll
-            for (int kk = 1; kk < 8; ++kk) wgmma_ss<32, 1, 1>(dqa, desc_adv(dsdesc, kk * 128), desc_adv(kdesc_mn, kk * 128), 1u);
+        for (int kk = 0; kk < 4; ++kk) wgmma_rs<SW, 1>(dk, da[kk], desc_adv(qdesc_mn, kk * 128), 1u);
+        if (wg == 0) {
+            if (dq_cols) {
+#pragma unroll
+                for (int kk = 0; kk < 8; ++kk) wgmma_ss<H0, 1, 1>(dqa, desc_adv(dsdesc, kk * 128), desc_adv(kdesc_mn, kk * 128), kk ? 1u : 0u);
+            }
+        } else if (dq_cols) {
+#pragma unroll
+            for (int kk = 0; kk < 8; ++kk) wgmma_ss<H1A, 1, 1>(dqa_a, desc_adv(dsdesc, kk * 128), desc_adv(kdesc_mn, kk * 128), kk ? 1u : 0u);
+            if constexpr (H1B > 0) {
+                if (p.col0 + 64 < p.d) {
+#pragma unroll
+                    for (int kk = 0; kk < 8; ++kk)
+                        wgmma_ss<H1B, 1, 1>(dqa_b, desc_adv(dsdesc, kk * 128), desc_adv(kdesc_mn_b, kk * 128), kk ? 1u : 0u);
+                }
+            }
         }
         wgmma_commit();
         wgmma_wait<0>();
         wgmma_fence_acc(dv);
         wgmma_fence_acc(dk);
         wgmma_fence_acc(dqa);
+        wgmma_fence_acc(dqa_a);
+        wgmma_fence_acc(dqa_b);
+        ATTN_TRACE(6);
         asm volatile("bar.sync 1, 256;" ::: "memory");
         if (threadIdx.x == 0 && i + STAGES < i1) load_q(i + STAGES);
+        ATTN_TRACE(7);
         if (!dq_cols) continue;
-#pragma unroll
-        for (int hh = 0; hh < 2; ++hh) {
-            const int q = i * 64 + r0 + 8 * hh;
-            if (q >= p.Lq) continue;
-#pragma unroll
-            for (int c8 = 0; c8 < 4; ++c8) {
-                const int col = dq_col + 8 * c8 + cq;
-                if (col < p.d) red_add_v2(p.dq_acc + ((bh * (p.dq_ld / 4) + col / 4) * p.Lq + q) * 4 + (col & 3), dqa[4 * c8 + 2 * hh], dqa[4 * c8 + 2 * hh + 1]);
-            }
-        }
-    }
+        auto drain = [&](const auto& acc, int c0) {
+            constexpr int n8 = sizeof(acc) / (4 * sizeof(float));
+#pragma unroll
+            for (int hh = 0; hh < 2; ++hh) {
+                const int q = i * 64 + r0 + 8 * hh;
+                if (q >= p.Lq) continue;
+#pragma unroll
+                for (int c8 = 0; c8 < n8; ++c8) {
+                    const int col = c0 + 8 * c8 + cq;
+                    if (col < p.d)
+                        red_add_v2(p.dq_acc + ((bh * (p.dq_ld / 4) + col / 4) * p.Lq + q) * 4 + (col & 3), acc[4 * c8 + 2 * hh], acc[4 * c8 + 2 * hh + 1]);
+                }
+            }
+        };
+        if (wg == 0) {
+            drain(dqa, dq_col);
+        } else {
+            drain(dqa_a, dq_col);
+            if constexpr (H1B > 0) drain(dqa_b, p.col0 + 64);
+        }
+    }
+    ATTN_TRACE(8);
+    ATTN_TRACE_FLUSH(1, i1 - i0);
 #pragma unroll
     for (int hh = 0; hh < 2; ++hh) {
         if (!kv_ok[hh]) continue;
         const int kv = kvw + r0 + 8 * hh;
 #pragma unroll
-        for (int c8 = 0; c8 < 8; ++c8) {
+        for (int c8 = 0; c8 < SW / 8; ++c8) {
             const int col = p.col0 + 8 * c8 + cq;
             if (col >= p.d) continue;
             const float v0 = dv[4 * c8 + 2 * hh], v1 = dv[4 * c8 + 2 * hh + 1];
@@ -491,31 +618,31 @@
     return HCP_OK;
 }
 
-template <int NB, int KVT, bool kCausal>
+template <int NB, int KVT, int DN, bool kCausal>
 static int launch_attn_fwd(const AttnFwdParams& p, dim3 grid, cudaStream_t stream) {
     using Cfg = AttnFwdCfg<NB, KVT>;
     static bool configured = false;
     if (!configured) {
-        cudaError_t e = cudaFuncSetAttribute(attn_fwd_kernel<NB, KVT, kCausal>, cudaFuncAttributeMaxDynamicSharedMemorySize, Cfg::SMEM_BYTES);
+        cudaError_t e = cudaFuncSetAttribute(attn_fwd_kernel<NB, KVT, DN, kCausal>, cudaFuncAttributeMaxDynamicSharedMemorySize, Cfg::SMEM_BYTES);
         if (e != cudaSuccess) return set_cuda_error(e, "cudaFuncSetAttribute(attn_fwd)");
         configured = true;
     }
-    launch_k(attn_fwd_kernel<NB, KVT, kCausal>, grid, dim3(kAttnThreads), Cfg::SMEM_BYTES, stream, p);
+    launch_k(attn_fwd_kernel<NB, KVT, DN, kCausal>, grid, dim3(kAttnThreads), Cfg::SMEM_BYTES, stream, p);
     cudaError_t e = cudaGetLastError();
     if (e != cudaSuccess) return set_cuda_error(e, "attn_fwd launch");
     return HCP_OK;
 }
 
-template <int NB, bool kCausal>
+template <int NB, int SW, bool kCausal>
 static int launch_attn_bwd(const AttnBwdParams& p, dim3 grid, cudaStream_t stream) {
     using Cfg = AttnBwdCfg<NB>;
     static bool configured = false;
     if (!configured) {
-        cudaError_t e = cudaFuncSetAttribute(attn_bwd_kernel<NB, kCausal>, cudaFuncAttributeMaxDynamicSharedMemorySize, Cfg::SMEM_BYTES);
+        cudaError_t e = cudaFuncSetAttribute(attn_bwd_kernel<NB, SW, kCausal>, cudaFuncAttributeMaxDynamicSharedMemorySize, Cfg::SMEM_BYTES);
         if (e != cudaSuccess) return set_cuda_error(e, "cudaFuncSetAttribute(attn_bwd)");
         configured = true;
     }
-    launch_k(attn_bwd_kernel<NB, kCausal>, grid, dim3(kAttnBwdThreads), Cfg::SMEM_BYTES, stream, p);
+    launch_k(attn_bwd_kernel<NB, SW, kCausal>, grid, dim3(kAttnBwdThreads), Cfg::SMEM_BYTES, stream, p);
     cudaError_t e = cudaGetLastError();
     if (e != cudaSuccess) return set_cuda_error(e, "attn_bwd launch");
     return HCP_OK;
@@ -546,9 +673,12 @@
     p.lse = a->lse;
     const dim3 grid((unsigned)((a->Lq + 127) / 128), (unsigned)a->H, (unsigned)a->B);
     cudaStream_t stream = (cudaStream_t)stream_;
-    if (nb == 1) return launch_attn_fwd<1, 128, kCausal>(p, grid, stream);
-    if (nb == 2) return launch_attn_fwd<2, 128, kCausal>(p, grid, stream);
-    return launch_attn_fwd<3, 64, kCausal>(p, grid, stream);
+    if (a->d <= 40) return launch_attn_fwd<1, 128, 40, kCausal>(p, grid, stream);
+    if (a->d <= 64) return launch_attn_fwd<1, 128, 64, kCausal>(p, grid, stream);
+    if (a->d <= 80) return launch_attn_fwd<2, 128, 80, kCausal>(p, grid, stream);
+    if (a->d <= 128) return launch_attn_fwd<2, 128, 128, kCausal>(p, grid, stream);
+    if (a->d <= 160) return launch_attn_fwd<3, 64, 160, kCausal>(p, grid, stream);
+    return launch_attn_fwd<3, 64, 192, kCausal>(p, grid, stream);
 }
 
 extern "C" int hcp_attn_fwd_bf16(const hcp_attn_args* a, hcp_stream_t stream) { return attn_fwd<false>(a, stream); }
@@ -617,12 +747,22 @@
     p.dV = (__nv_bfloat16*)a->dv; p.lddv = a->lddv;
     const int nb = (int)((a->d + 63) / 64);
     const dim3 grid((unsigned)(((a->Lkv + 127) / 128) * qsplit), (unsigned)a->H, (unsigned)a->B);
-    for (int col0 = 0; col0 < a->d; col0 += 64) {
-        p.col0 = col0;
-        rc = nb == 1 ? launch_attn_bwd<1, kCausal>(p, grid, stream) : nb == 2 ? launch_attn_bwd<2, kCausal>(p, grid, stream)
-                     : launch_attn_bwd<3, kCausal>(p, grid, stream);
-        if (rc) return rc;
-    }
+    if (a->d <= 40) {
+        p.col0 = 0;
+        rc = launch_attn_bwd<1, 40, kCausal>(p, grid, stream);
+    } else if (a->d <= 64) {
+        p.col0 = 0;
+        rc = launch_attn_bwd<1, 64, kCausal>(p, grid, stream);
+    } else if (a->d <= 80) {
+        p.col0 = 0;
+        rc = launch_attn_bwd<2, 80, kCausal>(p, grid, stream);
+    } else {
+        for (int col0 = 0; col0 < a->d && !rc; col0 += 64) {
+            p.col0 = col0;
+            rc = nb == 2 ? launch_attn_bwd<2, 64, kCausal>(p, grid, stream) : launch_attn_bwd<3, 64, kCausal>(p, grid, stream);
+        }
+    }
+    if (rc) return rc;
     {
         const int64_t n = a->B * a->Lq * a->H * (a->d / 4);
         launch_k(attn_bwd_post_kernel, dim3((unsigned)((n + 255) / 256)), dim3(256), 0, stream, dq_acc, dq_ld, (int)a->B, (int)a->H, (int)a->Lq,
@@ -640,3 +780,14 @@
 
 extern "C" int hcp_attn_bwd_bf16(const hcp_attn_bwd_args* a, hcp_stream_t stream) { return attn_bwd<false>(a, stream); }
 extern "C" int hcp_attn_bwd_causal_bf16(const hcp_attn_bwd_args* a, hcp_stream_t stream) { return attn_bwd<true>(a, stream); }
+
+#ifdef HCP_ATTN_TRACE
+extern "C" int hcp_attn_trace_read(unsigned long long* out) {
+    cudaError_t e = cudaMemcpyFromSymbol(out, g_attn_trace, sizeof(g_attn_trace));
+    if (e == cudaSuccess) {
+        static const unsigned long long zero[2][kTracePhases + 1] = {};
+        e = cudaMemcpyToSymbol(g_attn_trace, zero, sizeof(zero));
+    }
+    return e == cudaSuccess ? HCP_OK : set_cuda_error(e, "hcp_attn_trace_read");
+}
+#endif
diff --git a/hcp_diffusion_b200/csrc/wgmma.cuh b/hcp_diffusion_b200/csrc/wgmma.cuh
--- a/hcp_diffusion_b200/csrc/wgmma.cuh
+++ b/hcp_diffusion_b200/csrc/wgmma.cuh
@@ -2,97 +2,99 @@
 #include <stdint.h>
 
 namespace hcp {
-template <int TA, int TB>
-__device__ __forceinline__ void wgmma_ss_n32(float (&d)[16], uint64_t a, uint64_t b, uint32_t accumulate) {
-    asm volatile(
-        "{\n\t.reg .pred p;\n\t"
-        "setp.ne.b32 p, %18, 0;\n\t"
-        "wgmma.mma_async.sync.aligned.m64n32k16.f32.bf16.bf16 "
-        "{%0, %1, %2, %3, %4, %5, %6, %7, %8, %9, %10, %11, %12, %13, %14, %15}, "
-        "%16, %17, p, 1, 1, %19, %20;\n\t}"
-        : "+f"(d[0]), "+f"(d[1]), "+f"(d[2]), "+f"(d[3]), "+f"(d[4]), "+f"(d[5]), "+f"(d[6]), "+f"(d[7]), "+f"(d[8]), "+f"(d[9]), "+f"(d[10]), "+f"(d[11]), "+f"(d[12]), "+f"(d[13]), "+f"(d[14]), "+f"(d[15])
-        : "l"(a), "l"(b), "r"(accumulate), "n"(TA), "n"(TB));
-}
-template <int TA, int TB>
-__device__ __forceinline__ void wgmma_ss_n64(float (&d)[32], uint64_t a, uint64_t b, uint32_t accumulate) {
-    asm volatile(
-        "{\n\t.reg .pred p;\n\t"
-        "setp.ne.b32 p, %34, 0;\n\t"
-        "wgmma.mma_async.sync.aligned.m64n64k16.f32.bf16.bf16 "
-        "{%0, %1, %2, %3, %4, %5, %6, %7, %8, %9, %10, %11, %12, %13, %14, %15, %16, %17, %18, %19, %20, %21, %22, %23, %24, %25, %26, %27, %28, %29, %30, %31}, "
-        "%32, %33, p, 1, 1, %35, %36;\n\t}"
-        : "+f"(d[0]), "+f"(d[1]), "+f"(d[2]), "+f"(d[3]), "+f"(d[4]), "+f"(d[5]), "+f"(d[6]), "+f"(d[7]), "+f"(d[8]), "+f"(d[9]), "+f"(d[10]), "+f"(d[11]), "+f"(d[12]), "+f"(d[13]), "+f"(d[14]), "+f"(d[15]), "+f"(d[16]), "+f"(d[17]), "+f"(d[18]), "+f"(d[19]), "+f"(d[20]), "+f"(d[21]), "+f"(d[22]), "+f"(d[23]), "+f"(d[24]), "+f"(d[25]), "+f"(d[26]), "+f"(d[27]), "+f"(d[28]), "+f"(d[29]), "+f"(d[30]), "+f"(d[31])
-        : "l"(a), "l"(b), "r"(accumulate), "n"(TA), "n"(TB));
-}
-template <int TA, int TB>
-__device__ __forceinline__ void wgmma_ss_n128(float (&d)[64], uint64_t a, uint64_t b, uint32_t accumulate) {
-    asm volatile(
-        "{\n\t.reg .pred p;\n\t"
-        "setp.ne.b32 p, %66, 0;\n\t"
-        "wgmma.mma_async.sync.aligned.m64n128k16.f32.bf16.bf16 "
-        "{%0, %1, %2, %3, %4, %5, %6, %7, %8, %9, %10, %11, %12, %13, %14, %15, %16, %17, %18, %19, %20, %21, %22, %23, %24, %25, %26, %27, %28, %29, %30, %31, %32, %33, %34, %35, %36, %37, %38, %39, %40, %41, %42, %43, %44, %45, %46, %47, %48, %49, %50, %51, %52, %53, %54, %55, %56, %57, %58, %59, %60, %61, %62, %63}, "
-        "%64, %65, p, 1, 1, %67, %68;\n\t}"
-        : "+f"(d[0]), "+f"(d[1]), "+f"(d[2]), "+f"(d[3]), "+f"(d[4]), "+f"(d[5]), "+f"(d[6]), "+f"(d[7]), "+f"(d[8]), "+f"(d[9]), "+f"(d[10]), "+f"(d[11]), "+f"(d[12]), "+f"(d[13]), "+f"(d[14]), "+f"(d[15]), "+f"(d[16]), "+f"(d[17]), "+f"(d[18]), "+f"(d[19]), "+f"(d[20]), "+f"(d[21]), "+f"(d[22]), "+f"(d[23]), "+f"(d[24]), "+f"(d[25]), "+f"(d[26]), "+f"(d[27]), "+f"(d[28]), "+f"(d[29]), "+f"(d[30]), "+f"(d[31]), "+f"(d[32]), "+f"(d[33]), "+f"(d[34]), "+f"(d[35]), "+f"(d[36]), "+f"(d[37]), "+f"(d[38]), "+f"(d[39]), "+f"(d[40]), "+f"(d[41]), "+f"(d[42]), "+f"(d[43]), "+f"(d[44]), "+f"(d[45]), "+f"(d[46]), "+f"(d[47]), "+f"(d[48]), "+f"(d[49]), "+f"(d[50]), "+f"(d[51]), "+f"(d[52]), "+f"(d[53]), "+f"(d[54]), "+f"(d[55]), "+f"(d[56]), "+f"(d[57]), "+f"(d[58]), "+f"(d[59]), "+f"(d[60]), "+f"(d[61]), "+f"(d[62]), "+f"(d[63])
-        : "l"(a), "l"(b), "r"(accumulate), "n"(TA), "n"(TB));
-}
-template <int TA, int TB>
-__device__ __forceinline__ void wgmma_ss_n160(float (&d)[80], uint64_t a, uint64_t b, uint32_t accumulate) {
-    asm volatile(
-        "{\n\t.reg .pred p;\n\t"
-        "setp.ne.b32 p, %82, 0;\n\t"
-        "wgmma.mma_async.sync.aligned.m64n160k16.f32.bf16.bf16 "
-        "{%0, %1, %2, %3, %4, %5, %6, %7, %8, %9, %10, %11, %12, %13, %14, %15, %16, %17, %18, %19, %20, %21, %22, %23, %24, %25, %26, %27, %28, %29, %30, %31, %32, %33, %34, %35, %36, %37, %38, %39, %40, %41, %42, %43, %44, %45, %46, %47, %48, %49, %50, %51, %52, %53, %54, %55, %56, %57, %58, %59, %60, %61, %62, %63, %64, %65, %66, %67, %68, %69, %70, %71, %72, %73, %74, %75, %76, %77, %78, %79}, "
-        "%80, %81, p, 1, 1, %83, %84;\n\t}"
-        : "+f"(d[0]), "+f"(d[1]), "+f"(d[2]), "+f"(d[3]), "+f"(d[4]), "+f"(d[5]), "+f"(d[6]), "+f"(d[7]), "+f"(d[8]), "+f"(d[9]), "+f"(d[10]), "+f"(d[11]), "+f"(d[12]), "+f"(d[13]), "+f"(d[14]), "+f"(d[15]), "+f"(d[16]), "+f"(d[17]), "+f"(d[18]), "+f"(d[19]), "+f"(d[20]), "+f"(d[21]), "+f"(d[22]), "+f"(d[23]), "+f"(d[24]), "+f"(d[25]), "+f"(d[26]), "+f"(d[27]), "+f"(d[28]), "+f"(d[29]), "+f"(d[30]), "+f"(d[31]), "+f"(d[32]), "+f"(d[33]), "+f"(d[34]), "+f"(d[35]), "+f"(d[36]), "+f"(d[37]), "+f"(d[38]), "+f"(d[39]), "+f"(d[40]), "+f"(d[41]), "+f"(d[42]), "+f"(d[43]), "+f"(d[44]), "+f"(d[45]), "+f"(d[46]), "+f"(d[47]), "+f"(d[48]), "+f"(d[49]), "+f"(d[50]), "+f"(d[51]), "+f"(d[52]), "+f"(d[53]), "+f"(d[54]), "+f"(d[55]), "+f"(d[56]), "+f"(d[57]), "+f"(d[58]), "+f"(d[59]), "+f"(d[60]), "+f"(d[61]), "+f"(d[62]), "+f"(d[63]), "+f"(d[64]), "+f"(d[65]), "+f"(d[66]), "+f"(d[67]), "+f"(d[68]), "+f"(d[69]), "+f"(d[70]), "+f"(d[71]), "+f"(d[72]), "+f"(d[73]), "+f"(d[74]), "+f"(d[75]), "+f"(d[76]), "+f"(d[77]), "+f"(d[78]), "+f"(d[79])
-        : "l"(a), "l"(b), "r"(accumulate), "n"(TA), "n"(TB));
-}
-template <int TA, int TB>
-__device__ __forceinline__ void wgmma_ss_n176(float (&d)[88], uint64_t a, uint64_t b, uint32_t accumulate) {
-    asm volatile(
-        "{\n\t.reg .pred p;\n\t"
-        "setp.ne.b32 p, %90, 0;\n\t"
-        "wgmma.mma_async.sync.aligned.m64n176k16.f32.bf16.bf16 "
-        "{%0, %1, %2, %3, %4, %5, %6, %7, %8, %9, %10, %11, %12, %13, %14, %15, %16, %17, %18, %19, %20, %21, %22, %23, %24, %25, %26, %27, %28, %29, %30, %31, %32, %33, %34, %35, %36, %37, %38, %39, %40, %41, %42, %43, %44, %45, %46, %47, %48, %49, %50, %51, %52, %53, %54, %55, %56, %57, %58, %59, %60, %61, %62, %63, %64, %65, %66, %67, %68, %69, %70, %71, %72, %73, %74, %75, %76, %77, %78, %79, %80, %81, %82, %83, %84, %85, %86, %87}, "
-        "%88, %89, p, 1, 1, %91, %92;\n\t}"
-        : "+f"(d[0]), "+f"(d[1]), "+f"(d[2]), "+f"(d[3]), "+f"(d[4]), "+f"(d[5]), "+f"(d[6]), "+f"(d[7]), "+f"(d[8]), "+f"(d[9]), "+f"(d[10]), "+f"(d[11]), "+f"(d[12]), "+f"(d[13]), "+f"(d[14]), "+f"(d[15]), "+f"(d[16]), "+f"(d[17]), "+f"(d[18]), "+f"(d[19]), "+f"(d[20]), "+f"(d[21]), "+f"(d[22]), "+f"(d[23]), "+f"(d[24]), "+f"(d[25]), "+f"(d[26]), "+f"(d[27]), "+f"(d[28]), "+f"(d[29]), "+f"(d[30]), "+f"(d[31]), "+f"(d[32]), "+f"(d[33]), "+f"(d[34]), "+f"(d[35]), "+f"(d[36]), "+f"(d[37]), "+f"(d[38]), "+f"(d[39]), "+f"(d[40]), "+f"(d[41]), "+f"(d[42]), "+f"(d[43]), "+f"(d[44]), "+f"(d[45]), "+f"(d[46]), "+f"(d[47]), "+f"(d[48]), "+f"(d[49]), "+f"(d[50]), "+f"(d[51]), "+f"(d[52]), "+f"(d[53]), "+f"(d[54]), "+f"(d[55]), "+f"(d[56]), "+f"(d[57]), "+f"(d[58]), "+f"(d[59]), "+f"(d[60]), "+f"(d[61]), "+f"(d[62]), "+f"(d[63]), "+f"(d[64]), "+f"(d[65]), "+f"(d[66]), "+f"(d[67]), "+f"(d[68]), "+f"(d[69]), "+f"(d[70]), "+f"(d[71]), "+f"(d[72]), "+f"(d[73]), "+f"(d[74]), "+f"(d[75]), "+f"(d[76]), "+f"(d[77]), "+f"(d[78]), "+f"(d[79]), "+f"(d[80]), "+f"(d[81]), "+f"(d[82]), "+f"(d[83]), "+f"(d[84]), "+f"(d[85]), "+f"(d[86]), "+f"(d[87])
-        : "l"(a), "l"(b), "r"(accumulate), "n"(TA), "n"(TB));
-}
-template <int TB>
-__device__ __forceinline__ void wgmma_rs_n64(float (&d)[32], const uint32_t (&a)[4], uint64_t b, uint32_t accumulate) {
-    asm volatile(
-        "{\n\t.reg .pred p;\n\t"
-        "setp.ne.b32 p, %37, 0;\n\t"
-        "wgmma.mma_async.sync.aligned.m64n64k16.f32.bf16.bf16 "
-        "{%0, %1, %2, %3, %4, %5, %6, %7, %8, %9, %10, %11, %12, %13, %14, %15, %16, %17, %18, %19, %20, %21, %22, %23, %24, %25, %26, %27, %28, %29, %30, %31}, "
-        "{%32, %33, %34, %35}, %36, p, 1, 1, %38;\n\t}"
-        : "+f"(d[0]), "+f"(d[1]), "+f"(d[2]), "+f"(d[3]), "+f"(d[4]), "+f"(d[5]), "+f"(d[6]), "+f"(d[7]), "+f"(d[8]), "+f"(d[9]), "+f"(d[10]), "+f"(d[11]), "+f"(d[12]), "+f"(d[13]), "+f"(d[14]), "+f"(d[15]), "+f"(d[16]), "+f"(d[17]), "+f"(d[18]), "+f"(d[19]), "+f"(d[20]), "+f"(d[21]), "+f"(d[22]), "+f"(d[23]), "+f"(d[24]), "+f"(d[25]), "+f"(d[26]), "+f"(d[27]), "+f"(d[28]), "+f"(d[29]), "+f"(d[30]), "+f"(d[31])
-        : "r"(a[0]), "r"(a[1]), "r"(a[2]), "r"(a[3]), "l"(b), "r"(accumulate), "n"(TB));
-}
-template <int TB>
-__device__ __forceinline__ void wgmma_rs_n128(float (&d)[64], const uint32_t (&a)[4], uint64_t b, uint32_t accumulate) {
-    asm volatile(
-        "{\n\t.reg .pred p;\n\t"
-        "setp.ne.b32 p, %69, 0;\n\t"
-        "wgmma.mma_async.sync.aligned.m64n128k16.f32.bf16.bf16 "
-        "{%0, %1, %2, %3, %4, %5, %6, %7, %8, %9, %10, %11, %12, %13, %14, %15, %16, %17, %18, %19, %20, %21, %22, %23, %24, %25, %26, %27, %28, %29, %30, %31, %32, %33, %34, %35, %36, %37, %38, %39, %40, %41, %42, %43, %44, %45, %46, %47, %48, %49, %50, %51, %52, %53, %54, %55, %56, %57, %58, %59, %60, %61, %62, %63}, "
-        "{%64, %65, %66, %67}, %68, p, 1, 1, %70;\n\t}"
-        : "+f"(d[0]), "+f"(d[1]), "+f"(d[2]), "+f"(d[3]), "+f"(d[4]), "+f"(d[5]), "+f"(d[6]), "+f"(d[7]), "+f"(d[8]), "+f"(d[9]), "+f"(d[10]), "+f"(d[11]), "+f"(d[12]), "+f"(d[13]), "+f"(d[14]), "+f"(d[15]), "+f"(d[16]), "+f"(d[17]), "+f"(d[18]), "+f"(d[19]), "+f"(d[20]), "+f"(d[21]), "+f"(d[22]), "+f"(d[23]), "+f"(d[24]), "+f"(d[25]), "+f"(d[26]), "+f"(d[27]), "+f"(d[28]), "+f"(d[29]), "+f"(d[30]), "+f"(d[31]), "+f"(d[32]), "+f"(d[33]), "+f"(d[34]), "+f"(d[35]), "+f"(d[36]), "+f"(d[37]), "+f"(d[38]), "+f"(d[39]), "+f"(d[40]), "+f"(d[41]), "+f"(d[42]), "+f"(d[43]), "+f"(d[44]), "+f"(d[45]), "+f"(d[46]), "+f"(d[47]), "+f"(d[48]), "+f"(d[49]), "+f"(d[50]), "+f"(d[51]), "+f"(d[52]), "+f"(d[53]), "+f"(d[54]), "+f"(d[55]), "+f"(d[56]), "+f"(d[57]), "+f"(d[58]), "+f"(d[59]), "+f"(d[60]), "+f"(d[61]), "+f"(d[62]), "+f"(d[63])
-        : "r"(a[0]), "r"(a[1]), "r"(a[2]), "r"(a[3]), "l"(b), "r"(accumulate), "n"(TB));
-}
-template <int TB>
-__device__ __forceinline__ void wgmma_rs_n192(float (&d)[96], const uint32_t (&a)[4], uint64_t b, uint32_t accumulate) {
-    asm volatile(
-        "{\n\t.reg .pred p;\n\t"
-        "setp.ne.b32 p, %101, 0;\n\t"
-        "wgmma.mma_async.sync.aligned.m64n192k16.f32.bf16.bf16 "
-        "{%0, %1, %2, %3, %4, %5, %6, %7, %8, %9, %10, %11, %12, %13, %14, %15, %16, %17, %18, %19, %20, %21, %22, %23, %24, %25, %26, %27, %28, %29, %30, %31, %32, %33, %34, %35, %36, %37, %38, %39, %40, %41, %42, %43, %44, %45, %46, %47, %48, %49, %50, %51, %52, %53, %54, %55, %56, %57, %58, %59, %60, %61, %62, %63, %64, %65, %66, %67, %68, %69, %70, %71, %72, %73, %74, %75, %76, %77, %78, %79, %80, %81, %82, %83, %84, %85, %86, %87, %88, %89, %90, %91, %92, %93, %94, %95}, "
-        "{%96, %97, %98, %99}, %100, p, 1, 1, %102;\n\t}"
-        : "+f"(d[0]), "+f"(d[1]), "+f"(d[2]), "+f"(d[3]), "+f"(d[4]), "+f"(d[5]), "+f"(d[6]), "+f"(d[7]), "+f"(d[8]), "+f"(d[9]), "+f"(d[10]), "+f"(d[11]), "+f"(d[12]), "+f"(d[13]), "+f"(d[14]), "+f"(d[15]), "+f"(d[16]), "+f"(d[17]), "+f"(d[18]), "+f"(d[19]), "+f"(d[20]), "+f"(d[21]), "+f"(d[22]), "+f"(d[23]), "+f"(d[24]), "+f"(d[25]), "+f"(d[26]), "+f"(d[27]), "+f"(d[28]), "+f"(d[29]), "+f"(d[30]), "+f"(d[31]), "+f"(d[32]), "+f"(d[33]), "+f"(d[34]), "+f"(d[35]), "+f"(d[36]), "+f"(d[37]), "+f"(d[38]), "+f"(d[39]), "+f"(d[40]), "+f"(d[41]), "+f"(d[42]), "+f"(d[43]), "+f"(d[44]), "+f"(d[45]), "+f"(d[46]), "+f"(d[47]), "+f"(d[48]), "+f"(d[49]), "+f"(d[50]), "+f"(d[51]), "+f"(d[52]), "+f"(d[53]), "+f"(d[54]), "+f"(d[55]), "+f"(d[56]), "+f"(d[57]), "+f"(d[58]), "+f"(d[59]), "+f"(d[60]), "+f"(d[61]), "+f"(d[62]), "+f"(d[63]), "+f"(d[64]), "+f"(d[65]), "+f"(d[66]), "+f"(d[67]), "+f"(d[68]), "+f"(d[69]), "+f"(d[70]), "+f"(d[71]), "+f"(d[72]), "+f"(d[73]), "+f"(d[74]), "+f"(d[75]), "+f"(d[76]), "+f"(d[77]), "+f"(d[78]), "+f"(d[79]), "+f"(d[80]), "+f"(d[81]), "+f"(d[82]), "+f"(d[83]), "+f"(d[84]), "+f"(d[85]), "+f"(d[86]), "+f"(d[87]), "+f"(d[88]), "+f"(d[89]), "+f"(d[90]), "+f"(d[91]), "+f"(d[92]), "+f"(d[93]), "+f"(d[94]), "+f"(d[95])
-        : "r"(a[0]), "r"(a[1]), "r"(a[2]), "r"(a[3]), "l"(b), "r"(accumulate), "n"(TB));
-}
+
+#define HCP_WG_S4 "%0, %1, %2, %3"
+#define HCP_WG_O4 "+f"(d[0]), "+f"(d[1]), "+f"(d[2]), "+f"(d[3])
+#define HCP_WG_S8 HCP_WG_S4 ", %4, %5, %6, %7"
+#define HCP_WG_O8 HCP_WG_O4, "+f"(d[4]), "+f"(d[5]), "+f"(d[6]), "+f"(d[7])
+#define HCP_WG_S12 HCP_WG_S8 ", %8, %9, %10, %11"
+#define HCP_WG_O12 HCP_WG_O8, "+f"(d[8]), "+f"(d[9]), "+f"(d[10]), "+f"(d[11])
+#define HCP_WG_S16 HCP_WG_S12 ", %12, %13, %14, %15"
+#define HCP_WG_O16 HCP_WG_O12, "+f"(d[12]), "+f"(d[13]), "+f"(d[14]), "+f"(d[15])
+#define HCP_WG_S20 HCP_WG_S16 ", %16, %17, %18, %19"
+#define HCP_WG_O20 HCP_WG_O16, "+f"(d[16]), "+f"(d[17]), "+f"(d[18]), "+f"(d[19])
+#define HCP_WG_S24 HCP_WG_S20 ", %20, %21, %22, %23"
+#define HCP_WG_O24 HCP_WG_O20, "+f"(d[20]), "+f"(d[21]), "+f"(d[22]), "+f"(d[23])
+#define HCP_WG_S28 HCP_WG_S24 ", %24, %25, %26, %27"
+#define HCP_WG_O28 HCP_WG_O24, "+f"(d[24]), "+f"(d[25]), "+f"(d[26]), "+f"(d[27])
+#define HCP_WG_S32 HCP_WG_S28 ", %28, %29, %30, %31"
+#define HCP_WG_O32 HCP_WG_O28, "+f"(d[28]), "+f"(d[29]), "+f"(d[30]), "+f"(d[31])
+#define HCP_WG_S36 HCP_WG_S32 ", %32, %33, %34, %35"
+#define HCP_WG_O36 HCP_WG_O32, "+f"(d[32]), "+f"(d[33]), "+f"(d[34]), "+f"(d[35])
+#define HCP_WG_S40 HCP_WG_S36 ", %36, %37, %38, %39"
+#define HCP_WG_O40 HCP_WG_O36, "+f"(d[36]), "+f"(d[37]), "+f"(d[38]), "+f"(d[39])
+#define HCP_WG_S44 HCP_WG_S40 ", %40, %41, %42, %43"
+#define HCP_WG_O44 HCP_WG_O40, "+f"(d[40]), "+f"(d[41]), "+f"(d[42]), "+f"(d[43])
+#define HCP_WG_S48 HCP_WG_S44 ", %44, %45, %46, %47"
+#define HCP_WG_O48 HCP_WG_O44, "+f"(d[44]), "+f"(d[45]), "+f"(d[46]), "+f"(d[47])
+#define HCP_WG_S52 HCP_WG_S48 ", %48, %49, %50, %51"
+#define HCP_WG_O52 HCP_WG_O48, "+f"(d[48]), "+f"(d[49]), "+f"(d[50]), "+f"(d[51])
+#define HCP_WG_S56 HCP_WG_S52 ", %52, %53, %54, %55"
+#define HCP_WG_O56 HCP_WG_O52, "+f"(d[52]), "+f"(d[53]), "+f"(d[54]), "+f"(d[55])
+#define HCP_WG_S60 HCP_WG_S56 ", %56, %57, %58, %59"
+#define HCP_WG_O60 HCP_WG_O56, "+f"(d[56]), "+f"(d[57]), "+f"(d[58]), "+f"(d[59])
+#define HCP_WG_S64 HCP_WG_S60 ", %60, %61, %62, %63"
+#define HCP_WG_O64 HCP_WG_O60, "+f"(d[60]), "+f"(d[61]), "+f"(d[62]), "+f"(d[63])
+#define HCP_WG_S68 HCP_WG_S64 ", %64, %65, %66, %67"
+#define HCP_WG_O68 HCP_WG_O64, "+f"(d[64]), "+f"(d[65]), "+f"(d[66]), "+f"(d[67])
+#define HCP_WG_S72 HCP_WG_S68 ", %68, %69, %70, %71"
+#define HCP_WG_O72 HCP_WG_O68, "+f"(d[68]), "+f"(d[69]), "+f"(d[70]), "+f"(d[71])
+#define HCP_WG_S76 HCP_WG_S72 ", %72, %73, %74, %75"
+#define HCP_WG_O76 HCP_WG_O72, "+f"(d[72]), "+f"(d[73]), "+f"(d[74]), "+f"(d[75])
+#define HCP_WG_S80 HCP_WG_S76 ", %76, %77, %78, %79"
+#define HCP_WG_O80 HCP_WG_O76, "+f"(d[76]), "+f"(d[77]), "+f"(d[78]), "+f"(d[79])
+#define HCP_WG_S84 HCP_WG_S80 ", %80, %81, %82, %83"
+#define HCP_WG_O84 HCP_WG_O80, "+f"(d[80]), "+f"(d[81]), "+f"(d[82]), "+f"(d[83])
+#define HCP_WG_S88 HCP_WG_S84 ", %84, %85, %86, %87"
+#define HCP_WG_O88 HCP_WG_O84, "+f"(d[84]), "+f"(d[85]), "+f"(d[86]), "+f"(d[87])
+#define HCP_WG_S92 HCP_WG_S88 ", %88, %89, %90, %91"
+#define HCP_WG_O92 HCP_WG_O88, "+f"(d[88]), "+f"(d[89]), "+f"(d[90]), "+f"(d[91])
+#define HCP_WG_S96 HCP_WG_S92 ", %92, %93, %94, %95"
+#define HCP_WG_O96 HCP_WG_O92, "+f"(d[92]), "+f"(d[93]), "+f"(d[94]), "+f"(d[95])
+
+
+#define HCP_WGMMA_SS(N, R, OA, OB, OP, OTA, OTB)                                                                                  \
+    template <int TA, int TB>                                                                                                      \
+    __device__ __forceinline__ void wgmma_ss_n##N(float (&d)[R], uint64_t a, uint64_t b, uint32_t accumulate) {                    \
+        asm volatile("{\n\t.reg .pred p;\n\tsetp.ne.b32 p, %" #OP ", 0;\n\t"                                                      \
+                     "wgmma.mma_async.sync.aligned.m64n" #N "k16.f32.bf16.bf16 {" HCP_WG_S##R "}, %" #OA ", %" #OB               \
+                     ", p, 1, 1, %" #OTA ", %" #OTB ";\n\t}"                                                                      \
+                     : HCP_WG_O##R                                                                                                \
+                     : "l"(a), "l"(b), "r"(accumulate), "n"(TA), "n"(TB));                                                        \
+    }
+#define HCP_WGMMA_RS(N, R, OA0, OA1, OA2, OA3, OB, OP, OTB)                                                                       \
+    template <int TB>                                                                                                              \
+    __device__ __forceinline__ void wgmma_rs_n##N(float (&d)[R], const uint32_t (&a)[4], uint64_t b, uint32_t accumulate) {        \
+        asm volatile("{\n\t.reg .pred p;\n\tsetp.ne.b32 p, %" #OP ", 0;\n\t"                                                      \
+                     "wgmma.mma_async.sync.aligned.m64n" #N "k16.f32.bf16.bf16 {" HCP_WG_S##R "}, {%" #OA0 ", %" #OA1 ", %" #OA2   \
+                     ", %" #OA3 "}, %" #OB ", p, 1, 1, %" #OTB ";\n\t}"                                                           \
+                     : HCP_WG_O##R                                                                                                \
+                     : "r"(a[0]), "r"(a[1]), "r"(a[2]), "r"(a[3]), "l"(b), "r"(accumulate), "n"(TB));                             \
+    }
+
+HCP_WGMMA_SS(8, 4, 4, 5, 6, 7, 8)
+HCP_WGMMA_SS(16, 8, 8, 9, 10, 11, 12)
+HCP_WGMMA_SS(24, 12, 12, 13, 14, 15, 16)
+HCP_WGMMA_SS(32, 16, 16, 17, 18, 19, 20)
+HCP_WGMMA_SS(40, 20, 20, 21, 22, 23, 24)
+HCP_WGMMA_SS(64, 32, 32, 33, 34, 35, 36)
+HCP_WGMMA_SS(128, 64, 64, 65, 66, 67, 68)
+HCP_WGMMA_SS(160, 80, 80, 81, 82, 83, 84)
+HCP_WGMMA_SS(176, 88, 88, 89, 90, 91, 92)
+HCP_WGMMA_RS(40, 20, 20, 21, 22, 23, 24, 25, 26)
+HCP_WGMMA_RS(64, 32, 32, 33, 34, 35, 36, 37, 38)
+HCP_WGMMA_RS(80, 40, 40, 41, 42, 43, 44, 45, 46)
+HCP_WGMMA_RS(128, 64, 64, 65, 66, 67, 68, 69, 70)
+HCP_WGMMA_RS(160, 80, 80, 81, 82, 83, 84, 85, 86)
+HCP_WGMMA_RS(192, 96, 96, 97, 98, 99, 100, 101, 102)
+
 template <int N, int TA, int TB>
 __device__ __forceinline__ void wgmma_ss(float (&d)[N / 2], uint64_t a, uint64_t b, uint32_t accumulate) {
-    if constexpr (N == 32) wgmma_ss_n32<TA, TB>(d, a, b, accumulate);
+    if constexpr (N == 8) wgmma_ss_n8<TA, TB>(d, a, b, accumulate);
+    else if constexpr (N == 16) wgmma_ss_n16<TA, TB>(d, a, b, accumulate);
+    else if constexpr (N == 24) wgmma_ss_n24<TA, TB>(d, a, b, accumulate);
+    else if constexpr (N == 32) wgmma_ss_n32<TA, TB>(d, a, b, accumulate);
+    else if constexpr (N == 40) wgmma_ss_n40<TA, TB>(d, a, b, accumulate);
     else if constexpr (N == 64) wgmma_ss_n64<TA, TB>(d, a, b, accumulate);
     else if constexpr (N == 128) wgmma_ss_n128<TA, TB>(d, a, b, accumulate);
     else if constexpr (N == 160) wgmma_ss_n160<TA, TB>(d, a, b, accumulate);
@@ -101,8 +103,11 @@
 }
 template <int N, int TB>
 __device__ __forceinline__ void wgmma_rs(float (&d)[N / 2], const uint32_t (&a)[4], uint64_t b, uint32_t accumulate) {
-    if constexpr (N == 64) wgmma_rs_n64<TB>(d, a, b, accumulate);
+    if constexpr (N == 40) wgmma_rs_n40<TB>(d, a, b, accumulate);
+    else if constexpr (N == 64) wgmma_rs_n64<TB>(d, a, b, accumulate);
+    else if constexpr (N == 80) wgmma_rs_n80<TB>(d, a, b, accumulate);
     else if constexpr (N == 128) wgmma_rs_n128<TB>(d, a, b, accumulate);
+    else if constexpr (N == 160) wgmma_rs_n160<TB>(d, a, b, accumulate);
     else if constexpr (N == 192) wgmma_rs_n192<TB>(d, a, b, accumulate);
     else static_assert(N == 0, "wgmma_rs: unsupported N");
 }
```

Result: faster. 108.5, median of 6 (+3.2%).
